# LeCAR-Lab/dial-mpc

Hardware: AMD Instinct MI355X
Metric: sample-rollouts/sec (N x H env.steps), Go2 N=2048 H=16 (higher is better)
Workload: dtype f32

## Files before the change

### dial_mpc_amd/_lib.py

```python
from __future__ import annotations

import ctypes
import glob
import os
import subprocess
from typing import Optional

import numpy as np

from dial_mpc_amd import _abi

_CSRC = os.path.join(os.path.dirname(os.path.abspath(__file__)), "csrc")
LIB_PATH = os.environ.get("DIAL_HIP_LIB", os.path.join(_CSRC, "libdialhip.so"))
_lib = None


class DialHipError(RuntimeError):
    pass


IEEE_LIB_PATH = os.path.join(_CSRC, "libdialhip_ieee.so")


N_FAMILIES = 8
_FAST = ["-DDIAL_FUSED_DPP", "-fno-hip-fp32-correctly-rounded-divide-sqrt", "-Xarch_device", "-freciprocal-math", "-Xarch_device", "-fapprox-func",
         "-Xarch_device", "-fno-honor-nans"]
_IEEE = ["-Xarch_device", "-ffp-contract=off", "-DDIAL_IEEE_BUILD"]
_COMMON = ["--offload-arch=gfx950", "-O3", "-std=c++17", "-fPIC", "-Xarch_device", "-fno-slp-vectorize"]
_FAMILY_FLAGS = {3: ["-mllvm", "-amdgpu-sched-strategy=max-ilp"], 4: ["-mllvm", "-simplifycfg-sink-common=false"]}


def build(force: bool = False, verbose: bool = False, ieee: bool = False) -> str:
    if not ieee:
        build_plant(force=force, verbose=verbose)
        build_plant_dist(force=force, verbose=verbose)
        build_plant_var(force=force, verbose=verbose)
        build_plan_var(force=force, verbose=verbose)
        build_plan_ens(force=force, verbose=verbose)
    return _build_lib(IEEE_LIB_PATH if ieee else LIB_PATH, [(os.path.join(_CSRC, "dial_hip.hip"), [], "dial_hip.o")] +
                      [(os.path.join(_CSRC, "kern_family.hip"), [f"-DDIAL_FAMILY={k}"] + _FAMILY_FLAGS.get(k, []), f"kern_family_{k}.o")
                       for k in range(N_FAMILIES)], force, verbose, ieee)


PLANT_LIB_PATH = os.path.join(_CSRC, "libdialplant.so")
N_PLANT_FAMILIES = 7


def build_plant(force: bool = False, verbose: bool = False) -> str:
    return _build_lib(PLANT_LIB_PATH, [(os.path.join(_CSRC, "plant_family.hip"), [f"-DDIAL_FAMILY={k}"] + _FAMILY_FLAGS.get(k, []),
                                        f"plant_family_{k}.o") for k in range(N_PLANT_FAMILIES)], force, verbose, False)


PLANT_DIST_LIB_PATH = os.path.join(_CSRC, "libdialplantdist.so")


def build_plant_dist(force: bool = False, verbose: bool = False) -> str:
    return _build_lib(PLANT_DIST_LIB_PATH, [(os.path.join(_CSRC, "plant_dist_family.hip"), [f"-DDIAL_FAMILY={k}"] + _FAMILY_FLAGS.get(k, []),
                                             f"plant_dist_family_{k}.o") for k in range(N_PLANT_FAMILIES)], force, verbose, False)


PLANT_VAR_LIB_PATH = os.path.join(_CSRC, "libdialplantvar.so")


def build_plant_var(force: bool = False, verbose: bool = False) -> str:
    return _build_lib(PLANT_VAR_LIB_PATH, [(os.path.join(_CSRC, "plant_var_family.hip"), [f"-DDIAL_FAMILY={k}"] + _FAMILY_FLAGS.get(k, []),
                                            f"plant_var_family_{k}.o") for k in range(N_PLANT_FAMILIES)], force, verbose, False)


PLAN_VAR_LIB_PATH = os.path.join(_CSRC, "libdialplanvar.so")


def build_plan_var(force: bool = False, verbose: bool = False) -> str:
    return _build_lib(PLAN_VAR_LIB_PATH, [(os.path.join(_CSRC, "plan_var_family.hip"), [f"-DDIAL_FAMILY={k}"] + _FAMILY_FLAGS.get(k, []),
                                           f"plan_var_family_{k}.o") for k in range(N_PLANT_FAMILIES)], force, verbose, False)


PLAN_ENS_LIB_PATH = os.path.join(_CSRC, "libdialplanens.so")


def build_plan_ens(force: bool = False, verbose: bool = False) -> str:
    return _build_lib(PLAN_ENS_LIB_PATH, [(os.path.join(_CSRC, "plan_ens_family.hip"), [f"-DDIAL_FAMILY={k}"] + _FAMILY_FLAGS.get(k, []),
                                           f"plan_ens_family_{k}.o") for k in range(N_PLANT_FAMILIES)] +
                      [(os.path.join(_CSRC, "plan_ens_aggregate.hip"), [], "plan_ens_aggregate.o")], force, verbose, False)


def _build_lib(out: str, units, force: bool, verbose: bool, ieee: bool) -> str:
    from concurrent.futures import ThreadPoolExecutor
    srcs = sorted(glob.glob(os.path.join(_CSRC, "*.h")) + glob.glob(os.path.join(_CSRC, "*.hip"))) + [_abi.HEADER, os.path.abspath(__file__)]
    if not force and os.path.exists(out) and all(os.path.getmtime(out) >= os.path.getmtime(s) for s in srcs):
        return out
    hipcc = os.environ.get("HIPCC", "/opt/rocm/bin/hipcc")
    flags = _COMMON + (_IEEE if ieee else _FAST) + ([] if ieee else os.environ.get("DIAL_HIPCC_EXTRA", "").split())
    import fcntl
    import hashlib
    import shutil
    build_root = os.path.join(os.path.dirname(os.path.dirname(_CSRC)), "build")
    os.makedirs(build_root, exist_ok=True)
    tag = hashlib.sha1(" ".join(flags).encode()).hexdigest()[:8]
    objdir = os.path.join(build_root, f"obj_{os.path.basename(out)}_{tag}_{os.getpid()}")
    tmp_out = f"{out}.{os.getpid()}.tmp"
    with open(os.path.join(build_root, os.path.basename(out) + ".lock"), "w") as lock:
        fcntl.flock(lock, fcntl.LOCK_EX)
        try:
            if not force and os.path.exists(out) and all(os.path.getmtime(out) >= os.path.getmtime(s) for s in srcs):
                return out
            os.makedirs(objdir, exist_ok=True)
            units = [(src, defs, os.path.join(objdir, obj)) for src, defs, obj in units]

            def compile_unit(u):
                src, defs, obj = u
                cmd = [hipcc] + flags + defs + ["-c", "-o", obj, src]
                if verbose:
                    print(" ".join(cmd))
                r = subprocess.run(cmd, stdout=subprocess.PIPE, stderr=subprocess.STDOUT, text=True)
                if r.returncode != 0:
                    raise DialHipError(f"hipcc failed ({r.returncode}) on {os.path.basename(src)} {' '.join(defs)}:\n{r.stdout[-4000:]}")
                return obj
            with ThreadPoolExecutor(max_workers=min(len(units), os.cpu_count() or 1, 16)) as pool:
                objs = list(pool.map(compile_unit, units))
            cmd = [hipcc, "--offload-arch=gfx950", "-shared", "-fPIC", "-o", tmp_out] + objs
            if verbose:
                print(" ".join(cmd))
            subprocess.check_call(cmd)
            os.replace(tmp_out, out)
            return out
        finally:
            shutil.rmtree(objdir, ignore_errors=True)
            if os.path.exists(tmp_out):
                os.remove(tmp_out)
            fcntl.flock(lock, fcntl.LOCK_UN)


def load(path: Optional[str] = None):
    global _lib
    if path is None and _lib is not None:
        return _lib
    lib_path = LIB_PATH if path is None else path
    if not os.path.exists(lib_path):
        raise DialHipError(f"{lib_path} is missing: run `python -c 'import __graft_entry__ as g; g.build()'` "
                           "(the HIP extension is the only compute path; there is no CPU fallback)")
    lib = ctypes.CDLL(lib_path)
    vp, ci, fp = ctypes.c_void_p, ctypes.c_int, ctypes.c_void_p
    lib.dial_create.argtypes = [ctypes.POINTER(vp), vp, vp, vp, ci]
    lib.dial_create_sharded.argtypes = [ctypes.POINTER(vp), vp, vp, vp, ci, ci]
    lib.dial_create_ex.argtypes = [ctypes.POINTER(vp), vp, vp, vp, ci, ci, vp]
    lib.dial_set_state_trace.argtypes = [vp, fp, ci]
    lib.dial_destroy.argtypes = [vp]
    lib.dial_destroy.restype = None
    lib.dial_last_error.argtypes = [vp]
    lib.dial_last_error.restype = ctypes.c_char_p
    lib.dial_rollout.argtypes = [vp, fp, fp, ci, fp, fp, fp, fp, vp]
    lib.dial_reverse_once.argtypes = [vp, fp, fp, fp, ci, fp, fp, fp, fp, fp, fp, vp]
    lib.dial_shard_rollout.argtypes = [vp, fp, fp, fp, ci, fp, ci, ci, fp, vp]
    lib.dial_shard_reduce.argtypes = [vp, fp, ci, ci, ci, ci, fp, vp]
    lib.dial_shard_ybar.argtypes = [vp, fp, ci, fp, fp, fp, ci, fp, vp]
    u64, u32 = ctypes.c_uint64, ctypes.c_uint32
    lib.dial_reverse_once_rng.argtypes = [vp, fp, fp, fp, ci, u64, u32, fp, fp, fp, fp, fp, vp]
# ... 570 lines not shown
        Y = Y.clone()
        self._check(self.lib.dial_shift_batch(self.h, _ptr(Y), int(Y.shape[0]), _stream()), "dial_shift_batch")
        return Y

    def rng_fill(self, seed: int, counter: int, n_begin: int, n_count: int):
        import torch
        eps = torch.empty((n_count, self.cfg.Hnode + 1, self.nu), dtype=torch.float32, device=self.torch_device)
        self._check(self.lib.dial_rng_fill(self.h, int(seed), int(counter), n_begin, n_count, _ptr(eps), _stream()),
                    "dial_rng_fill")
        return eps

    def shard_rollout_rng(self, state, Ybar, noise_scale, seed, counter, n_begin, n_local, with_mean, rews_local):
        self._check(self.lib.dial_shard_rollout_rng(self.h, _ptr(state), _ptr(Ybar), _ptr(noise_scale),
                                                    int(noise_scale.numel()), int(seed), int(counter), n_begin, n_local,
                                                    int(with_mean), _ptr(rews_local), _stream()), "dial_shard_rollout_rng")

    def shard_rollout(self, state, Ybar, noise_scale, eps_local, n_local: int, with_mean: bool, rews_local):
        ns = int(noise_scale.numel())
        self._check(self.lib.dial_shard_rollout(self.h, _ptr(state), _ptr(Ybar), _ptr(noise_scale), ns,
                                                _ptr(eps_local) if n_local > 0 else None, n_local, int(with_mean),
                                                _ptr(rews_local), _stream()), "dial_shard_rollout")

    def shard_reduce(self, rews_all, n_total: int, n_begin: int, n_local: int, include_mean: bool, packed_out):
        self._check(self.lib.dial_shard_reduce(self.h, _ptr(rews_all), n_total, n_begin, n_local, int(include_mean),
                                               _ptr(packed_out), _stream()), "dial_shard_reduce")

    def shard_ybar(self, rews_all, n_total: int, eps_all, Ybar, noise_scale, Ybar_out):
        ns = int(noise_scale.numel())
        self._check(self.lib.dial_shard_ybar(self.h, _ptr(rews_all), n_total, _ptr(eps_all), _ptr(Ybar), _ptr(noise_scale),
                                             ns, _ptr(Ybar_out), _stream()), "dial_shard_ybar")

    def shard_ybar_rng(self, rews_all, n_total: int, seed: int, counter: int, Ybar, noise_scale, Ybar_out):
        self._check(self.lib.dial_shard_ybar_rng(self.h, _ptr(rews_all), n_total, int(seed), int(counter), _ptr(Ybar),
                                                 _ptr(noise_scale), int(noise_scale.numel()), _ptr(Ybar_out), _stream()),
                    "dial_shard_ybar_rng")

    def shard_pack_rewards(self, gathered, world: int, per: int, n_total: int, rews_all):
        self._check(self.lib.dial_shard_pack_rewards(self.h, _ptr(gathered), world, per, n_total, _ptr(rews_all), _stream()),
                    "dial_shard_pack_rewards")

    def shard_ybar_gathered(self, gathered, world: int, per: int, n_total: int, eps_all, Ybar, noise_scale, rews_all, Ybar_out):
        self._check(self.lib.dial_shard_ybar_gathered(self.h, _ptr(gathered), world, per, n_total, _ptr(eps_all), _ptr(Ybar), _ptr(noise_scale),
                                                      int(noise_scale.numel()), _ptr(rews_all), _ptr(Ybar_out), _stream()), "dial_shard_ybar_gathered")

    def shard_ybar_gathered_rng(self, gathered, world: int, per: int, n_total: int, seed: int, counter: int, Ybar, noise_scale, rews_all, Ybar_out):
        self._check(self.lib.dial_shard_ybar_gathered_rng(self.h, _ptr(gathered), world, per, n_total, int(seed), int(counter), _ptr(Ybar),
                                                          _ptr(noise_scale), int(noise_scale.numel()), _ptr(rews_all), _ptr(Ybar_out), _stream()),
                    "dial_shard_ybar_gathered_rng")

    def shard_reduce_gathered(self, gathered, world: int, per: int, n_total: int, n_begin: int, n_local: int, include_mean: bool, rews_all, packed_out):
        self._check(self.lib.dial_shard_reduce_gathered(self.h, _ptr(gathered), world, per, n_total, n_begin, n_local, int(include_mean),
                                                        _ptr(rews_all), _ptr(packed_out), _stream()), "dial_shard_reduce_gathered")

    def packed_size(self) -> int:
        T, Hn1 = self.cfg.Hsample + 1, self.cfg.Hnode + 1
        return Hn1 * self.nu + T * (self.nq + self.nv + self.nx)

    def shift(self, Y):
        Y = Y.clone()
        self._check(self.lib.dial_shift(self.h, _ptr(Y), _stream()), "dial_shift")
        return Y

    def status(self):
        self._check(self.lib.dial_status(self.h), "dial_status")

    def set_timing(self, enable: bool):
        self._check(self.lib.dial_set_timing(self.h, int(enable)), "dial_set_timing")

    def rollout_ms(self):
        tot, n = ctypes.c_double(0), ctypes.c_int(0)
        self._check(self.lib.dial_get_rollout_ms(self.h, ctypes.byref(tot), ctypes.byref(n)), "dial_get_rollout_ms")
        return tot.value, n.value

    def set_state_trace(self, rows: Optional[int]):
        import torch
        if rows is None:
            self._check(self.lib.dial_set_state_trace(self.h, None, 0), "dial_set_state_trace")
            self._trace = None
            return None
        self._trace = torch.zeros((int(rows), self.cfg.Hsample + 1, self.state_size), dtype=torch.float32, device=self.torch_device)
        self._check(self.lib.dial_set_state_trace(self.h, _ptr(self._trace), int(rows)), "dial_set_state_trace")
        return self._trace

    LAUNCH_FIELDS = ("inst", "wpb", "blocks", "queue", "relay", "mean_inline", "slice_pieces", "split", "pair", "trace", "con_cap", "rollouts")

    def debug_last_launch(self) -> dict:
        buf = (ctypes.c_int * len(self.LAUNCH_FIELDS))()
        n = self.lib.dial_debug_last_launch(self.h, buf, len(buf))
        if n != len(self.LAUNCH_FIELDS):
            raise DialHipError(f"dial_debug_last_launch: {n} fields, this wrapper knows {len(self.LAUNCH_FIELDS)}")
        return dict(zip(self.LAUNCH_FIELDS, buf))

    def debug_scratch(self):
        import numpy as np
        import torch
        ptrs = [ctypes.c_void_p() for _ in range(6)]
        self._check(self.lib.dial_debug_scratch(self.h, *[ctypes.byref(p) for p in ptrs]), "dial_debug_scratch")
        cfg = self.cfg
        B, T, Hn1 = cfg.Nsample + 1, cfg.Hsample + 1, cfg.Hnode + 1
        shapes = [(B, Hn1, self.nu), (B, T), (B, T, self.nq), (B, T, self.nv), (B, T, self.nx), (B,)]
        names = ["Y0s", "rewss", "qss", "qdss", "xss", "weights"]
        torch.cuda.synchronize()
        hip = ctypes.CDLL("libamdhip64.so")
        out = {}
        for name, p, shp in zip(names, ptrs, shapes):
            host = np.empty(shp, np.float32)
            rc = hip.hipMemcpy(host.ctypes.data_as(ctypes.c_void_p), p, ctypes.c_size_t(host.nbytes), ctypes.c_int(2))
            if rc != 0:
                raise DialHipError(f"hipMemcpy of scratch {name} failed ({rc})")
            out[name] = host
        return out
```

### dial_mpc_amd/csrc/dial_hip.hip

```cpp
#include <dlfcn.h>
#include <hip/hip_runtime.h>

#include <cstdio>
#include <cstdlib>
#include <cstring>
#include <string>
#include <vector>

#include "kernel_list.h"
#include "plant_kernel.h"
#include "plant_plugin.h"
#include "plant_dist_kernel.h"
#include "plant_var_kernel.h"
#include "plan_var_kernel.h"
#include "plan_ens_kernel.h"
#include "plugin_ops.h"

#define DIAL_X(D, WPB, OCC, Q, TR) \
  extern template __global__ void rollout_kernel<D, WPB, OCC, Q, TR>(const CModel<D>*, const dial_task*, const dial_cfg*, dial::RolloutIO, int, int, int*);
#define DIAL_XE(D)                                                                                                                                    \
  extern template __global__ void env_step_kernel<D>(const CModel<D>*, const dial_task*, float*, const float*, float*, float*, float*, const float*); \
  extern template __global__ void env_reset_kernel<D>(const CModel<D>*, const float*, const float*, float*, float*, float*);
DIAL_KERNELS_ALL(DIAL_X, DIAL_XE)
#define DIAL_X2(D, WPB, OCC, Q, MI) \
  extern template __global__ void rollout_kernel2<D, WPB, OCC, Q, MI>(const CModel<D>*, const dial_task*, const dial_cfg*, dial::RolloutIO, int, int, int*);
DIAL_KERNELS2_GO2(DIAL_X2)
#undef DIAL_X2
#undef DIAL_X
#undef DIAL_XE

#define WSUM_CHUNKS 64
#define YB_CHUNKS_HOST 128

#ifndef DIAL_GO2_LARGE_B
#define DIAL_GO2_LARGE_B 2304
#endif
#ifndef DIAL_GO2_PAIR_MIN_B
#define DIAL_GO2_PAIR_MIN_B 2304
#endif

#define WK_THREADS 1024
#ifndef DIAL_K4_FP64
#define DIAL_K4_FP64 0
#endif
__device__ __forceinline__ float block_sum(float v, float* red) {
  const int tid = threadIdx.x;
  float ws = dialwave::wave_sum_dpp(v);
  if ((tid & 63) == 0) red[tid >> 6] = ws;
  __syncthreads();
  float r = 0.f;
#pragma unroll
  for (int k = 0; k < WK_THREADS / 64; k++) r += red[k];
  __syncthreads();
  return r;
}
__device__ __forceinline__ double block_sum_d(double v, double* red) {
  const int tid = threadIdx.x;
  for (int o = 32; o > 0; o >>= 1) v += __shfl_xor(v, o, 64);
  if ((tid & 63) == 0) red[tid >> 6] = v;
  __syncthreads();
  double r = 0.0;
#pragma unroll
  for (int k = 0; k < WK_THREADS / 64; k++) r += red[k];
  __syncthreads();
  return r;
}
__device__ __forceinline__ float block_max(float v, float* red) {
  const int tid = threadIdx.x;
  float wm = dialwave::wave_max_shfl(v);
  if ((tid & 63) == 0) red[tid >> 6] = wm;
  __syncthreads();
  float r = -INFINITY;
#pragma unroll
  for (int k = 0; k < WK_THREADS / 64; k++) r = red[k] > r ? red[k] : r;
  __syncthreads();
  return r;
}

extern "C" __global__ void __launch_bounds__(WK_THREADS)
weights_kernel(const float* __restrict__ rews_in, int B, float temp, float* __restrict__ weights, const float* __restrict__ gathered,
               int per, float* __restrict__ rews_out) {
  __shared__ float red[WK_THREADS / 64];
  const int tid = threadIdx.x;
  const float* rews = rews_in + (size_t)blockIdx.x * B;
  weights += (size_t)blockIdx.x * B;
  if (gathered) {
    const int n_total = B - 1;
    for (int n = tid; n < B; n += WK_THREADS)
      rews_out[n] = n < n_total ? gathered[(size_t)(n / per) * (per + 1) + (n % per)] : gathered[per];
    __threadfence_block();
    __syncthreads();
    rews = rews_out;
  }
#if DIAL_K4_FP64
  __shared__ double redd[WK_THREADS / 64];
  double accd = 0.0;
  float mxr = -INFINITY;
  for (int n = tid; n < B; n += WK_THREADS) { float r = rews[n]; accd += (double)r; mxr = r > mxr ? r : mxr; }
  const double mean = block_sum_d(accd, redd) / (double)B;
// ... 103 lines not shown
        if (eps) {
#pragma unroll
          for (int e = 0; e < 4; e++) z[e] = c0 + e < C ? eps[(size_t)n * C + c0 + e] : 0.f;
        } else {
          dial::normal_quad((uint32_t)n, (uint32_t)q, iter, seed_lo, seed_hi, z);
        }
      }
      const float wn = weights[n];
#pragma unroll
      for (int e = 0; e < 4; e++) {
        float v = n < n_total ? (kk[e] == 0 ? y0[e] : z[e] * sc[e] + yb[e]) : yb[e];
        v = v < -1.f ? -1.f : (v > 1.f ? 1.f : v);
        acc[e] += wn * v;
      }
    }
  }
#pragma unroll
  for (int e = 0; e < 4; e++) red[rl][4 * ql + e] = acc[e];
  __syncthreads();
  const int cl = threadIdx.x, c = blockIdx.x * 64 + cl;
  if (cl < 64 && c < C) {
    float t = 0.f;
    for (int r = 0; r < 16; r++) t += red[r][cl];
    partial[(size_t)chunk * C + c] = t;
  }
}
extern "C" __global__ void __launch_bounds__(64)
ybar_final_kernel(const float* __restrict__ partial, int C, float* __restrict__ out) {
  const int c = blockIdx.x * 64 + threadIdx.x;
  if (c >= C) return;
  float acc = 0.f;
#pragma unroll 16
  for (int ch = 0; ch < YB_CHUNKS; ch++) acc += partial[(size_t)ch * C + c];
  out[c] = acc;
}

extern "C" __global__ void __launch_bounds__(256)
rng_fill_kernel(uint32_t seed_lo, uint32_t seed_hi, uint32_t iter, int n_begin, int n_count, int C, float* eps_out) {
  const int nq = (C + 3) / 4;
  const long long t = (long long)blockIdx.x * 256 + threadIdx.x;
  if (t >= (long long)n_count * nq) return;
  const int n = (int)(t / nq), q = (int)(t - (long long)n * nq);
  float z[4];
  dial::normal_quad((uint32_t)(n_begin + n), (uint32_t)q, iter, seed_lo, seed_hi, z);
  for (int e = 0; e < 4; e++)
    if (4 * q + e < C) eps_out[(size_t)n * C + 4 * q + e] = z[e];
}

extern "C" __global__ void __launch_bounds__(256)
pack_rewards_kernel(const float* __restrict__ gathered, int per, int n_total, float* __restrict__ rews_all) {
  const int n = blockIdx.x * 256 + threadIdx.x;
  if (n < n_total) rews_all[n] = gathered[(size_t)(n / per) * (per + 1) + (n % per)];
  else if (n == n_total) rews_all[n] = gathered[per];
}

extern "C" __global__ void __launch_bounds__(64)
shift_kernel(const dial_cfg* __restrict__ cfg, int nu, float* Y) {
  __shared__ float u[DIAL_MAX_T * DIAL_MAX_U];
  const int T = cfg->Hsample + 1, Hn1 = cfg->Hnode + 1;
  Y += (size_t)blockIdx.x * Hn1 * nu;
  for (int it = threadIdx.x; it < T * nu; it += 64) {
    const int st = it / nu, a = it - st * nu;
    float acc = 0.f;
    if (st + 1 < T)
      for (int k = 0; k < Hn1; k++) acc += cfg->W[st + 1][k] * Y[k * nu + a];
    u[it] = acc;
  }
  __syncthreads();
  for (int it = threadIdx.x; it < Hn1 * nu; it += 64) {
    const int k = it / nu, a = it - k * nu;
    float acc = 0.f;
    for (int st = 0; st < T; st++) acc += cfg->V[k][st] * u[st * nu + a];
    Y[it] = acc;
  }
}

extern "C" __global__ void __launch_bounds__(64) selftest_kernel(float* out) {
  float v = (float)threadIdx.x + 0.5f;
  float a = dialwave::wave_sum_dpp(v), b = dialwave::wave_sum_shfl(v), c = dialwave::wave_max_shfl(v);
  if (threadIdx.x == 0) { out[0] = a; out[1] = b; out[2] = c; }
}

enum LaunchField { LF_INST, LF_WPB, LF_BLOCKS, LF_QUEUE, LF_RELAY, LF_MEAN_INLINE, LF_SLICE_PIECES, LF_SPLIT, LF_PAIR, LF_TRACE, LF_CON_CAP,
                   LF_ROLLOUTS, DIAL_LAUNCH_FIELDS };

struct dial_ctx {
  int device = 0;
  dial_model hm;
  dial_task ht;
  dial_cfg hc;
  dial_derived hd;
  bool has_cfg = false;
  int inst = 0;
  const dial_plugin_ops* plug = nullptr;
  const dial_plugin_ctrl* plug_ctrl = nullptr;
  const dial_plugin_table* plug_table = nullptr;
  const dial_plugin_plant* plug_plant = nullptr;
  const dial_plugin_plant_dist* plug_plant_dist = nullptr;
  const float* plant_dist = nullptr;
  int plant_dist_M = 0, plant_dist_E = 0;
  const dial_plugin_plant_var* plug_plant_var = nullptr;
  void* plant_models = nullptr;
  int32_t* plant_model_of = nullptr;
  int plant_models_V = 0, plant_models_M = 0;
  const dial_plugin_plan_var* plug_plan_var = nullptr;
  void* plan_models = nullptr;
  int32_t* plan_model_of = nullptr;
  int plan_models_V = 0, plan_models_rows = 0, plan_models_mode = 0;
  dial_plan_var_launch_fn plan_launch = nullptr;
  const dial_plugin_plan_ens* plug_plan_ens = nullptr;
  void* ens_models = nullptr;
  int32_t* ens_hyp = nullptr;
  float* ens_raw = nullptr;
  int ens_V = 0, ens_rows = 0, ens_R = 0, ens_mode = 0, ens_k = 0;
  int ens_last_M = 0;
  dial_plan_ens_launch_fn ens_launch = nullptr;
  dial_plan_ens_aggregate_fn ens_aggregate = nullptr;
  std::vector<float> user_params;
  const float* user_table = nullptr;
  int user_table_rows = 0, user_table_cols = 0, user_table_row0 = 0, user_table_mode = 0;
  std::vector<char> plug_cm;
  const float* plan_params = nullptr;
  int plan_rows = 0;
  void* dcm = nullptr;
  size_t dcm_bytes = 0;
  dial_task* dtask = nullptr;
  dial_cfg* dcfg = nullptr;
  int con_cap = 0, ovf_words = 0;
  float* ovf = nullptr;
  int B_cap = 0, W_cap = 0, T = 0, Hn1 = 0, nx = 0;
  int plan_cap = 1;
  float *Y0s = nullptr, *rewss = nullptr, *rews = nullptr, *qss = nullptr, *qdss = nullptr, *xss = nullptr;
  float *weights = nullptr, *partial = nullptr;
  const char* rows_stale = nullptr;
  unsigned long long* prof = nullptr;
  size_t lds_bytes = 0;
  size_t lds_rollout = 0;
  size_t lds_large = 0;
  int ws_words = 0, cm_bytes = 0, wpb = 1;
  int* next = nullptr;
  float* relay_buf = nullptr;
  float* slice_buf = nullptr;
  int* slice_flag = nullptr;
  int slice_cap = 0, slice_stride = 0, slice_steps = 3;
  int* work_stat = nullptr;
  int* relay_flag = nullptr;
  int* err_host = nullptr;
  int* err_dev = nullptr;
  bool relay_ok = false, relay_always = false;
  bool no_spread = false;
  bool no_mean_inline = false;
  hipStream_t side = nullptr;
  hipEvent_t ev_fork = nullptr, ev_join = nullptr;
  size_t lds_even = 0, lds_one = 0;
  bool split_ok = false;
  int wpb_even = 0;
  int n_simd = 0;
  int debug_stall_piece1 = 0;
  int relay_steps = 3;
  int resident_blocks = 0, resident_blocks_large = 0;
  bool pair_ok = false;
  size_t lds_pair = 0, lds_pair_large = 0;
  int resident_pair = 0, resident_pair_large = 0;
  bool timing = false;
  dial_options opt{};
  float* trace = nullptr;
  int trace_rows = 0;
  int ovf_slots = 0;
  int last_launch[DIAL_LAUNCH_FIELDS] = {};
  std::vector<std::pair<hipEvent_t, hipEvent_t>> events;
  size_t events_used = 0;
  std::string err;
};

static thread_local std::string g_err;

static int fail(dial_ctx* ctx, int code, const std::string& msg) {
  if (ctx) ctx->err = msg;
  g_err = msg;
  return code;
}
#define HIP_TRY(ctx, expr)                                                                     \
  do {                                                                                         \
    hipError_t e_ = (expr);                                                                    \
    if (e_ != hipSuccess)                                                                      \
      return fail(ctx, DIAL_ERR_HIP, std::string(#expr) + ": " + hipGetErrorString(e_));       \
  } while (0)

template <class Tab>
static int plugin_table(void* h, const char* plugin_path, const char* symbol, const char* what, int version, const Tab** tab) {
  typedef const Tab* (*entry_fn)(void);
  *tab = nullptr;
  entry_fn entry = (entry_fn)dlsym(h, symbol);
  if (!entry) return DIAL_OK;
  *tab = entry();
  if (!*tab) return fail(nullptr, DIAL_ERR_ARG, std::string("dial_create_plugin: ") + plugin_path + ": " + symbol + " returned no table");
  if ((*tab)->version != version)
    return fail(nullptr, DIAL_ERR_ARG, std::string("dial_create_plugin: stale plugin: its ") + what + " reports version " + std::to_string((*tab)->version) +
                                       ", the library needs version " + std::to_string(version) + " (rebuild it from the current sources)");
  return DIAL_OK;
}

template <class D>
static void plant_model_block(void* dst, const dial_model* model, const dial_task* task, const dial_derived* dv) {
  CModel<D>* h = new CModel<D>();
  fill_cmodel(h, model, task, dv);
  memcpy(dst, h, sizeof(CModel<D>));
  delete h;
}

extern "C" {

const char* dial_last_error(const dial_ctx* ctx) { return ctx ? ctx->err.c_str() : g_err.c_str(); }

int dial_abi_sizes(int* a, int* b, int* c) {
  if (a) *a = (int)sizeof(dial_model);
  if (b) *b = (int)sizeof(dial_task);
  if (c) *c = (int)sizeof(dial_cfg);
  return DIAL_OK;
}

void dial_destroy(dial_ctx* ctx) {
  if (!ctx) return;
  (void)hipSetDevice(ctx->device);
  void* ptrs[] = {ctx->dcm, ctx->dtask, ctx->dcfg, ctx->prof, ctx->next, ctx->relay_buf, ctx->relay_flag, ctx->Y0s, ctx->rewss, ctx->rews, ctx->qss,
                  ctx->qdss,   ctx->xss,   ctx->weights, ctx->partial, ctx->ovf, ctx->slice_buf, ctx->slice_flag, ctx->work_stat,
                  ctx->plant_models, ctx->plant_model_of, ctx->plan_models, ctx->plan_model_of, ctx->ens_models, ctx->ens_hyp, ctx->ens_raw};
  for (void* p : ptrs)
    if (p) (void)hipFree(p);
  for (auto& ev : ctx->events) { (void)hipEventDestroy(ev.first); (void)hipEventDestroy(ev.second); }
  if (ctx->ev_fork) (void)hipEventDestroy(ctx->ev_fork);
  if (ctx->ev_join) (void)hipEventDestroy(ctx->ev_join);
  if (ctx->side) (void)hipStreamDestroy(ctx->side);
  if (ctx->err_host) (void)hipHostFree(ctx->err_host);
  delete ctx;
}

int dial_create(dial_ctx** out, const dial_model* model, const dial_task* task, const dial_cfg* cfg, int device) {
  return dial_create_ex(out, model, task, cfg, device, -1, nullptr);
}

int dial_create_sharded(dial_ctx** out, const dial_model* model, const dial_task* task, const dial_cfg* cfg, int device,
                        int n_local_cap) {
  if (cfg && (n_local_cap < 0 || n_local_cap > cfg->Nsample)) return fail(nullptr, DIAL_ERR_ARG, "dial_create_sharded: n_local_cap must be in [0, Nsample]");
  return dial_create_ex(out, model, task, cfg, device, n_local_cap, nullptr);
}

static int create_impl(dial_ctx** out, const dial_model* model, const dial_task* task, const dial_cfg* cfg, int device,
                       int n_local_cap, const dial_options* opts, const dial_plugin_ops* plug, const float* params, int n_params);

int dial_create_ex(dial_ctx** out, const dial_model* model, const dial_task* task, const dial_cfg* cfg, int device,
                   int n_local_cap, const dial_options* opts) {
  return create_impl(out, model, task, cfg, device, n_local_cap, opts, nullptr, nullptr, 0);
}

int dial_create_plugin(dial_ctx** out, const dial_model* model, const dial_task* task, const dial_cfg* cfg, int device,
                       const dial_options* opts, const char* plugin_path, const float* params, int n_params) {
  if (!out || !model || !task || !plugin_path) return fail(nullptr, DIAL_ERR_ARG, "dial_create_plugin: null argument");
// ... 310 lines not shown
      case 3: ctx->inst = 3; ctx->wpb = 2; urc = upload(DimsH1Loco{}); break;
      case 4: ctx->inst = 4; ctx->wpb = DIAL_ALLEGRO_WPB; urc = upload(DimsAllegro{}); break;
      case 5: ctx->inst = 5; ctx->wpb = DIAL_CRATE_WPB; urc = upload(DimsGo2Crate{}); break;
      case 6: ctx->inst = 6; ctx->wpb = DIAL_CRATE_WPB; urc = upload(DimsH1PushCrate{}); break;
      case 0: ctx->inst = 0; ctx->wpb = 1; urc = upload(DimsMax{}); break;
      default:
        dial_destroy(ctx);
        return fail(nullptr, DIAL_ERR_UNSUPPORTED, std::string("dial_create: elliptic-cone models need a dimension-specialised instantiation (built: Allegro hand)") +
                                                   (opt.force_generic ? "; options.force_generic does not apply to them" : ""));
    }
    if (urc != DIAL_OK) { dial_destroy(ctx); return fail(nullptr, urc, "dial_create: uploading the model constants failed"); }
    ctx->last_launch[LF_INST] = ctx->inst;
  }
  if (!cfg) ctx->lds_rollout = ctx->lds_bytes;
  if (ctx->lds_rollout > 160 * 1024 || ctx->lds_bytes > 64 * 1024) {
    dial_destroy(ctx);
    return fail(nullptr, DIAL_ERR_ARG, "dial_create: LDS workspace exceeds the 160 KiB of a CU");
  }
  if (ctx->inst == 1) ctx->lds_large = ctx->cm_bytes + (size_t)DIAL_GO2_WPB_LARGE * ctx->ws_words * sizeof(float);
  {
    hipError_t e = hipSuccess;
    if (ctx->inst == 4 && ctx->lds_rollout > 64 * 1024)
      e = hipFuncSetAttribute((const void*)rollout_kernel<DimsAllegro, DIAL_ALLEGRO_WPB>, hipFuncAttributeMaxDynamicSharedMemorySize, (int)ctx->lds_rollout);
    if (e == hipSuccess && ctx->inst == 4 && ctx->lds_rollout > 64 * 1024)
      e = hipFuncSetAttribute((const void*)rollout_kernel<DimsAllegro, DIAL_ALLEGRO_WPB, 3, true>, hipFuncAttributeMaxDynamicSharedMemorySize, (int)ctx->lds_rollout);
    if (e == hipSuccess && ctx->inst == 4 && ctx->lds_rollout > 64 * 1024)
      e = hipFuncSetAttribute((const void*)rollout_kernel<DimsAllegro, DIAL_ALLEGRO_WPB, 3, false, true>, hipFuncAttributeMaxDynamicSharedMemorySize, (int)ctx->lds_rollout);
#define DIAL_BIG_LDS(D)                                                                                                                         \
    if (e == hipSuccess && ctx->lds_rollout > 64 * 1024) {                                                                                     \
      e = hipFuncSetAttribute((const void*)rollout_kernel<D, DIAL_CRATE_WPB>, hipFuncAttributeMaxDynamicSharedMemorySize, (int)ctx->lds_rollout); \
      if (e == hipSuccess) e = hipFuncSetAttribute((const void*)rollout_kernel<D, DIAL_CRATE_WPB, 3, true>, hipFuncAttributeMaxDynamicSharedMemorySize, (int)ctx->lds_rollout); \
      if (e == hipSuccess) e = hipFuncSetAttribute((const void*)rollout_kernel<D, DIAL_CRATE_WPB, 3, false, true>, hipFuncAttributeMaxDynamicSharedMemorySize, (int)ctx->lds_rollout); \
    }
    if (ctx->inst == 7) e = ctx->plug->set_lds(ctx->lds_rollout);
    if (ctx->inst == 5) { DIAL_BIG_LDS(DimsGo2Crate) }
    if (ctx->inst == 6) { DIAL_BIG_LDS(DimsH1PushCrate) }
#undef DIAL_BIG_LDS
    if (e == hipSuccess && ctx->inst == 1 && ctx->lds_large > 64 * 1024)
      e = hipFuncSetAttribute((const void*)rollout_kernel<DimsGo2, DIAL_GO2_WPB_LARGE, DIAL_GO2_OCC_LARGE, true>, hipFuncAttributeMaxDynamicSharedMemorySize, (int)ctx->lds_large);
    if (ctx->inst == 1 && cfg) {
      ctx->pair_ok = opt.pair_mode != 1;
      ctx->lds_pair = ctx->cm_bytes + (size_t)2 * ctx->ws_words * sizeof(float);
      ctx->lds_pair_large = ctx->cm_bytes + (size_t)2 * DIAL_GO2_PAIR_WPB * ctx->ws_words * sizeof(float);
#ifdef DIAL_PROFILE
      ctx->lds_pair += 16 + 32 * sizeof(unsigned long long);
      ctx->lds_pair_large += 16 + (size_t)DIAL_GO2_PAIR_WPB * 32 * sizeof(unsigned long long);
#endif
      if (ctx->lds_pair_large > 160 * 1024) ctx->pair_ok = false;
      if (e == hipSuccess && ctx->pair_ok && ctx->lds_pair_large > 64 * 1024)
        e = hipFuncSetAttribute((const void*)rollout_kernel2<DimsGo2, DIAL_GO2_PAIR_WPB, DIAL_GO2_PAIR_OCC, true, true>, hipFuncAttributeMaxDynamicSharedMemorySize, (int)ctx->lds_pair_large);
    }
    if (e != hipSuccess) { dial_destroy(ctx); return fail(nullptr, DIAL_ERR_HIP, std::string("dial_create: hipFuncSetAttribute: ") + hipGetErrorString(e)); }
  }
  {
    hipDeviceProp_t prop;
    HIP_TRY_CREATE(hipGetDeviceProperties(&prop, device));
    int nb = 0;
    hipError_t e = hipSuccess;
#define DIAL_RESIDENT(D, WPB) e = hipOccupancyMaxActiveBlocksPerMultiprocessor(&nb, rollout_kernel<D, WPB>, 64 * WPB, ctx->lds_rollout)
    if (ctx->inst == 1) DIAL_RESIDENT(DimsGo2, 1);
    else if (ctx->inst == 2) DIAL_RESIDENT(DimsH1, 3);
    else if (ctx->inst == 3) DIAL_RESIDENT(DimsH1Loco, 2);
    else if (ctx->inst == 4) DIAL_RESIDENT(DimsAllegro, DIAL_ALLEGRO_WPB);
    else if (ctx->inst == 5) DIAL_RESIDENT(DimsGo2Crate, DIAL_CRATE_WPB);
    else if (ctx->inst == 6) DIAL_RESIDENT(DimsH1PushCrate, DIAL_CRATE_WPB);
    else if (ctx->inst == 7) e = ctx->plug->occupancy(&nb, ctx->lds_rollout);
    else DIAL_RESIDENT(DimsMax, 1);
#undef DIAL_RESIDENT
    ctx->n_simd = 4 * prop.multiProcessorCount;
    if (e == hipSuccess) ctx->resident_blocks = nb * prop.multiProcessorCount;
    if (e == hipSuccess && ctx->inst == 1) {
      e = hipOccupancyMaxActiveBlocksPerMultiprocessor(&nb, rollout_kernel<DimsGo2, DIAL_GO2_WPB_LARGE, DIAL_GO2_OCC_LARGE, true>,
                                                       64 * DIAL_GO2_WPB_LARGE, ctx->lds_large);
      if (e == hipSuccess) ctx->resident_blocks_large = nb * prop.multiProcessorCount;
    }
    if (e == hipSuccess && ctx->pair_ok) {
      e = hipOccupancyMaxActiveBlocksPerMultiprocessor(&nb, rollout_kernel2<DimsGo2, 1, DIAL_GO2_PAIR_OCC, false, false>, 64, ctx->lds_pair);
      if (e == hipSuccess) ctx->resident_pair = nb * prop.multiProcessorCount;
      if (e == hipSuccess) e = hipOccupancyMaxActiveBlocksPerMultiprocessor(&nb, rollout_kernel2<DimsGo2, DIAL_GO2_PAIR_WPB, DIAL_GO2_PAIR_OCC, true, true>,
                                                                            64 * DIAL_GO2_PAIR_WPB, ctx->lds_pair_large);
      if (e == hipSuccess) ctx->resident_pair_large = nb * prop.multiProcessorCount;
      if (e == hipSuccess && (ctx->resident_pair <= 0 || ctx->resident_pair_large <= 0)) ctx->pair_ok = false;
    }
    if (e != hipSuccess) { dial_destroy(ctx); return fail(nullptr, DIAL_ERR_HIP, std::string("dial_create: occupancy query: ") + hipGetErrorString(e)); }
    if (opt.no_queue) ctx->resident_blocks = ctx->resident_blocks_large = 0;
    HIP_TRY_CREATE(hipMalloc(&ctx->next, sizeof(int)));
    HIP_TRY_CREATE(hipMalloc(&ctx->relay_buf, sizeof(float) * (DIAL_MAX_Q + 2 * DIAL_MAX_V + DIAL_INFO_N + 4)));
    HIP_TRY_CREATE(hipMalloc(&ctx->relay_flag, sizeof(int)));
    HIP_TRY_CREATE(hipMemset(ctx->relay_flag, 0, sizeof(int)));
    HIP_TRY_CREATE(hipHostMalloc((void**)&ctx->err_host, sizeof(int), hipHostMallocMapped));
    *ctx->err_host = 0;
    HIP_TRY_CREATE(hipHostGetDevicePointer((void**)&ctx->err_dev, ctx->err_host, 0));
    ctx->relay_ok = ctx->wpb == 1 && !opt.no_relay;
    ctx->relay_always = opt.relay_always != 0;
    ctx->no_mean_inline = opt.no_mean_inline != 0;
    ctx->no_spread = opt.no_spread != 0;
    ctx->wpb_even = ctx->inst == 4 ? DIAL_ALLEGRO_WPB_EVEN : ctx->inst == 2 ? DIAL_H1_WPB_EVEN : 0;
    if ((opt.no_split_mask >> ctx->inst) & 1) ctx->wpb_even = 0;
    if (ctx->wpb_even > 0) {
      ctx->lds_even = ctx->cm_bytes + (size_t)ctx->wpb_even * ctx->ws_words * sizeof(float);
      ctx->lds_one = ctx->cm_bytes + (size_t)ctx->ws_words * sizeof(float);
#ifdef DIAL_PROFILE
      ctx->lds_even += 16 + (size_t)ctx->wpb_even * 32 * sizeof(unsigned long long);
      ctx->lds_one += 16 + 32 * sizeof(unsigned long long);
#endif
      if ((8 / ctx->wpb_even) * ctx->lds_even + ctx->lds_one <= 160 * 1024) {
        hipError_t e2 = hipSuccess;
        if (ctx->lds_even > 64 * 1024) {
          if (ctx->inst == 4) e2 = hipFuncSetAttribute((const void*)rollout_kernel<DimsAllegro, DIAL_ALLEGRO_WPB_EVEN, DIAL_EVEN_OCC_ALLEGRO>, hipFuncAttributeMaxDynamicSharedMemorySize, (int)ctx->lds_even);
          else e2 = hipFuncSetAttribute((const void*)rollout_kernel<DimsH1, DIAL_H1_WPB_EVEN, DIAL_EVEN_OCC_H1>, hipFuncAttributeMaxDynamicSharedMemorySize, (int)ctx->lds_even);
        }
        if (e2 == hipSuccess) e2 = hipStreamCreateWithFlags(&ctx->side, hipStreamNonBlocking);
        if (e2 == hipSuccess) e2 = hipEventCreateWithFlags(&ctx->ev_fork, hipEventDisableTiming);
        if (e2 == hipSuccess) e2 = hipEventCreateWithFlags(&ctx->ev_join, hipEventDisableTiming);
        if (e2 != hipSuccess) { dial_destroy(ctx); return fail(nullptr, DIAL_ERR_HIP, std::string("dial_create: split-launch set-up: ") + hipGetErrorString(e2)); }
        ctx->split_ok = true;
      }
    }
    if (opt.relay_steps >= 1) ctx->relay_steps = opt.relay_steps;
    ctx->debug_stall_piece1 = opt.debug_relay_stall;
  }
  HIP_TRY_CREATE(hipMalloc(&ctx->dtask, sizeof(dial_task)));
  HIP_TRY_CREATE(hipMemcpy(ctx->dtask, task, sizeof(dial_task), hipMemcpyHostToDevice));
  if (cfg) {
    if (cfg->Hsample + 1 > DIAL_MAX_T || cfg->Hnode + 1 > DIAL_MAX_NODE || cfg->Hnode < 2 || cfg->Nsample < 1) {
      dial_destroy(ctx);
      return fail(nullptr, DIAL_ERR_ARG, "dial_create: Hsample/Hnode/Nsample out of range");
    }
    ctx->hc = *cfg;
    ctx->has_cfg = true;
    ctx->B_cap = n_local_cap + 1;
    ctx->W_cap = cfg->Nsample + 1;
    ctx->ovf_slots = ctx->plan_cap * ctx->B_cap + (cfg->Hsample + 1 > 16 ? cfg->Hsample + 1 : 16);
    if (ctx->con_cap > 0) HIP_TRY_CREATE(hipMalloc(&ctx->ovf, (size_t)ctx->ovf_slots * ctx->ovf_words * sizeof(float)));
    ctx->T = cfg->Hsample + 1;
    ctx->Hn1 = cfg->Hnode + 1;
    if (ctx->inst == 4 && !opt.no_lag_priority) HIP_TRY_CREATE(hipMalloc(&ctx->work_stat, 2 * sizeof(int)));
    const int B_all = ctx->plan_cap * ctx->B_cap;
    if (ctx->inst == 4 && !opt.no_slice && ctx->resident_blocks > 0 && B_all > ctx->resident_blocks * ctx->wpb) {
      ctx->slice_stride = model->nq + 2 * model->nv + DIAL_INFO_N + 4;
      ctx->slice_cap = B_all;
      if (opt.slice_steps >= 1) ctx->slice_steps = opt.slice_steps;
      HIP_TRY_CREATE(hipMalloc(&ctx->slice_buf, sizeof(float) * (size_t)ctx->slice_stride * B_all));
      HIP_TRY_CREATE(hipMalloc(&ctx->slice_flag, sizeof(int) * (size_t)B_all));
      HIP_TRY_CREATE(hipMemset(ctx->slice_flag, 0, sizeof(int) * (size_t)B_all));
    }
    const size_t B = B_all, T = ctx->T;
    HIP_TRY_CREATE(hipMalloc(&ctx->dcfg, sizeof(dial_cfg)));
    HIP_TRY_CREATE(hipMemcpy(ctx->dcfg, cfg, sizeof(dial_cfg), hipMemcpyHostToDevice));
    HIP_TRY_CREATE(hipMalloc(&ctx->Y0s, sizeof(float) * B * ctx->Hn1 * model->nu));
    HIP_TRY_CREATE(hipMalloc(&ctx->rewss, sizeof(float) * B * T));
    HIP_TRY_CREATE(hipMalloc(&ctx->rews, sizeof(float) * ctx->W_cap));
    HIP_TRY_CREATE(hipMalloc(&ctx->qss, sizeof(float) * B * T * model->nq));
    HIP_TRY_CREATE(hipMalloc(&ctx->qdss, sizeof(float) * B * T * model->nv));
    HIP_TRY_CREATE(hipMalloc(&ctx->xss, sizeof(float) * B * T * ctx->nx));
    HIP_TRY_CREATE(hipMalloc(&ctx->weights, sizeof(float) * ctx->W_cap * ctx->plan_cap));
    const size_t Ctot = (size_t)ctx->Hn1 * model->nu + T * (model->nq + model->nv + ctx->nx);
    const size_t part_w = ((Ctot + 63) / 64) * (size_t)WSUM_CHUNKS * 64, part_y = (((size_t)ctx->Hn1 * model->nu + 63) / 64) * (size_t)YB_CHUNKS_HOST * 64;
    HIP_TRY_CREATE(hipMalloc(&ctx->partial, sizeof(float) * (part_w * ctx->plan_cap > part_y ? part_w * ctx->plan_cap : part_y)));
    HIP_TRY_CREATE(hipMalloc(&ctx->prof, sizeof(unsigned long long) * (32 + 6 * B)));
    HIP_TRY_CREATE(hipMemset(ctx->prof, 0, sizeof(unsigned long long) * (32 + 6 * B)));
  }
#undef HIP_TRY_CREATE
  *out = ctx;
  return DIAL_OK;
}
// ... 132 lines not shown
    if ((B + 1) / 2 <= ctx->resident_pair || opt_no_queue(ctx)) {
      const int pairs = (B + 1) / 2;
      ll[LF_PAIR] = 1; ll[LF_WPB] = 1; ll[LF_BLOCKS] = pairs;
      hipLaunchKernelGGL((rollout_kernel2<DimsGo2, 1, DIAL_GO2_PAIR_OCC, false, false>), dim3(pairs), dim3(64), ctx->lds_pair, st,
                         (const CModel<DimsGo2>*)ctx->dcm, (const dial_task*)ctx->dtask, (const dial_cfg*)ctx->dcfg, io, B, ctx->ws_words, (int*)nullptr);
    } else {
      const int blocks = ctx->resident_pair_large;
      if (mean_last && ctx->T <= blocks * DIAL_GO2_PAIR_WPB) {
        io.mean_inline = 1;
        io.relay_buf = ctx->relay_buf;
        io.relay_flag = ctx->relay_flag;
        io.err_word = ctx->err_dev;
      }
      HIP_TRY(ctx, hipMemsetD32Async((hipDeviceptr_t)ctx->next, blocks * DIAL_GO2_PAIR_WPB, 1, st));
      ll[LF_PAIR] = 1; ll[LF_WPB] = DIAL_GO2_PAIR_WPB; ll[LF_BLOCKS] = blocks; ll[LF_QUEUE] = 1; ll[LF_MEAN_INLINE] = io.mean_inline;
      hipLaunchKernelGGL((rollout_kernel2<DimsGo2, DIAL_GO2_PAIR_WPB, DIAL_GO2_PAIR_OCC, true, true>), dim3(blocks), dim3(64 * DIAL_GO2_PAIR_WPB),
                         ctx->lds_pair_large, st, (const CModel<DimsGo2>*)ctx->dcm, (const dial_task*)ctx->dtask, (const dial_cfg*)ctx->dcfg, io, B,
                         ctx->ws_words, ctx->next);
    }
    HIP_TRY(ctx, hipGetLastError());
    if (ctx->timing) HIP_TRY(ctx, hipEventRecord(e1, st));
    return DIAL_OK;
  }
  const bool large = ctx->inst == 1 && B > DIAL_GO2_LARGE_B && !tracing;
  const int wpb = large ? DIAL_GO2_WPB_LARGE : ctx->wpb;
  const int resident = large ? ctx->resident_blocks_large : ctx->resident_blocks;
  dial::RolloutIO io = io_in;
  io.plan_params = ctx->plan_params;
  io.con_cap = ctx->ovf ? ctx->con_cap : 0;
  io.ovf = ctx->ovf;
  io.ovf_words = ctx->ovf_words;
  bool relay = false;
  if (ctx->relay_ok && !large && !io.us && !io.plan_rollouts && io.n_noise == B - 1 && B > 1 && ctx->T >= 4 && ctx->n_simd > 0 &&
      ((B - 1) % ctx->n_simd == 0 || ctx->relay_always)) {
    const int pieces = (ctx->T + ctx->relay_steps - 1) / ctx->relay_steps;
    if ((B - 1) + pieces <= ctx->resident_blocks) {
      io.relay_buf = ctx->relay_buf;
      io.relay_flag = ctx->relay_flag;
      io.relay_steps = ctx->relay_steps;
      io.relay_base = B - 1;
      io.err_word = ctx->err_dev;
      io.debug_stall_piece1 = ctx->debug_stall_piece1;
      relay = true;
    }
  }
  int blocks = io.relay_flag ? io.relay_base + (ctx->T + io.relay_steps - 1) / io.relay_steps : (B + wpb - 1) / wpb;
  if (large && !io.relay_flag && resident > 0 && blocks < resident && !ctx->no_spread) {
    blocks = resident;
    io.spread = 1;
  }
  int* next = nullptr;
  const bool has_queue_variant = large || ctx->inst != 1;
  if (has_queue_variant && resident > 0 && blocks > resident && ctx->next && !tracing) {
    blocks = resident;
    next = ctx->next;
    HIP_TRY(ctx, hipMemsetD32Async((hipDeviceptr_t)next, blocks * wpb, 1, st));
    if (large && !ctx->no_mean_inline && !io.us && !io.plan_rollouts && io.n_noise == B - 1 && ctx->T <= blocks * wpb && io.relay_stride == 0) {
      io.mean_inline = 1;
      io.relay_buf = ctx->relay_buf;
      io.relay_flag = ctx->relay_flag;
      io.err_word = ctx->err_dev;
    }
    if (!io.mean_inline && ctx->slice_buf && B <= ctx->slice_cap && ctx->T > ctx->slice_steps) {
      io.relay_buf = ctx->slice_buf;
      io.relay_flag = ctx->slice_flag;
      io.relay_stride = ctx->slice_stride;
      io.relay_steps = ctx->slice_steps;
      io.slice_pieces = (ctx->T + ctx->slice_steps - 1) / ctx->slice_steps;
      io.err_word = ctx->err_dev;
    }
  }
  if (ctx->work_stat && !io.slice_pieces && !tracing) {
    HIP_TRY(ctx, hipMemsetAsync(ctx->work_stat, 0, 2 * sizeof(int), st));
    io.work_stat = ctx->work_stat;
  }
  if (io.ovf && blocks * wpb > ctx->ovf_slots)
    return fail(ctx, DIAL_ERR_ARG, "rollout launch: more wavefronts than overflow areas (batch larger than the context's Nsample + 1)");
  if (ctx->trace) {
    if (B > ctx->trace_rows) return fail(ctx, DIAL_ERR_ARG, "rollout launch: more rollouts than rows of the state trace (dial_set_state_trace)");
    io.trace = ctx->trace;
  }
  ll[LF_WPB] = wpb; ll[LF_BLOCKS] = blocks; ll[LF_QUEUE] = next != nullptr; ll[LF_RELAY] = relay; ll[LF_MEAN_INLINE] = io.mean_inline;
  ll[LF_SLICE_PIECES] = io.slice_pieces; ll[LF_TRACE] = tracing; ll[LF_CON_CAP] = io.con_cap;
  if (ctx->split_ok && !tracing && !next && !io.us && !io.plan_rollouts && io.n_noise == B - 1 && (B - 1) == 8 * (ctx->n_simd / 4)) {
    HIP_TRY(ctx, hipEventRecord(ctx->ev_fork, st));
    HIP_TRY(ctx, hipStreamWaitEvent(ctx->side, ctx->ev_fork, 0));
    dial::RolloutIO io1 = io;
    io1.n_first = B - 1;
    ll[LF_SPLIT] = 1; ll[LF_WPB] = ctx->wpb_even; ll[LF_BLOCKS] = (B - 1) / ctx->wpb_even;
#define DIAL_SPLIT_LAUNCH(D, WPBE, OCCE)                                                                                       \
    hipLaunchKernelGGL((rollout_kernel<D, 1>), dim3(1), dim3(64), ctx->lds_one, ctx->side, (const CModel<D>*)ctx->dcm,     \
                       (const dial_task*)ctx->dtask, (const dial_cfg*)ctx->dcfg, io1, B, ctx->ws_words, (int*)nullptr);    \
    HIP_TRY(ctx, hipGetLastError());                                                                                       \
    HIP_TRY(ctx, hipEventRecord(ctx->ev_join, ctx->side));                                                                 \
    hipLaunchKernelGGL((rollout_kernel<D, WPBE, OCCE>), dim3((B - 1) / WPBE), dim3(64 * WPBE), ctx->lds_even, st,                \
                       (const CModel<D>*)ctx->dcm, (const dial_task*)ctx->dtask, (const dial_cfg*)ctx->dcfg, io, B - 1,    \
                       ctx->ws_words, (int*)nullptr)
    if (ctx->inst == 4) { DIAL_SPLIT_LAUNCH(DimsAllegro, DIAL_ALLEGRO_WPB_EVEN, DIAL_EVEN_OCC_ALLEGRO); }
    else { DIAL_SPLIT_LAUNCH(DimsH1, DIAL_H1_WPB_EVEN, DIAL_EVEN_OCC_H1); }
#undef DIAL_SPLIT_LAUNCH
    HIP_TRY(ctx, hipGetLastError());
    HIP_TRY(ctx, hipStreamWaitEvent(st, ctx->ev_join, 0));
    if (ctx->timing) HIP_TRY(ctx, hipEventRecord(e1, st));
    return DIAL_OK;
  }
#define DIAL_LAUNCH_ROLLOUT_Q(D, WPB, Q)                                                                    \
  hipLaunchKernelGGL((rollout_kernel<D, WPB, 3, Q>), dim3(blocks), dim3(64 * WPB), ctx->lds_rollout,        \
                     st, (const CModel<D>*)ctx->dcm, (const dial_task*)ctx->dtask,                          \
                     (const dial_cfg*)ctx->dcfg, io, B, ctx->ws_words, next)
#define DIAL_LAUNCH_ROLLOUT(D, WPB)                                        \
  do {                                                                     \
    if (next) DIAL_LAUNCH_ROLLOUT_Q(D, WPB, true);                         \
    else DIAL_LAUNCH_ROLLOUT_Q(D, WPB, false);                             \
  } while (0)
#define DIAL_LAUNCH_TRACE(D, WPB)                                                                           \
  hipLaunchKernelGGL((rollout_kernel<D, WPB, 3, false, true>), dim3(blocks), dim3(64 * WPB), ctx->lds_rollout, \
                     st, (const CModel<D>*)ctx->dcm, (const dial_task*)ctx->dtask,                          \
                     (const dial_cfg*)ctx->dcfg, io, B, ctx->ws_words, (int*)nullptr)
  if (tracing) {
    if (ctx->inst == 1) DIAL_LAUNCH_TRACE(DimsGo2, 1);
    else if (ctx->inst == 2) DIAL_LAUNCH_TRACE(DimsH1, 3);
    else if (ctx->inst == 3) DIAL_LAUNCH_TRACE(DimsH1Loco, 2);
    else if (ctx->inst == 4) DIAL_LAUNCH_TRACE(DimsAllegro, DIAL_ALLEGRO_WPB);
    else if (ctx->inst == 5) DIAL_LAUNCH_TRACE(DimsGo2Crate, DIAL_CRATE_WPB);
    else if (ctx->inst == 6) DIAL_LAUNCH_TRACE(DimsH1PushCrate, DIAL_CRATE_WPB);
    else if (ctx->inst == 7) HIP_TRY(ctx, ctx->plug->rollout(2, blocks, ctx->lds_rollout, st, ctx->dcm, ctx->dtask, ctx->dcfg, &io, B, ctx->ws_words, nullptr));
    else DIAL_LAUNCH_TRACE(DimsMax, 1);
  } else
  if (large)
    hipLaunchKernelGGL((rollout_kernel<DimsGo2, DIAL_GO2_WPB_LARGE, DIAL_GO2_OCC_LARGE, true>), dim3(blocks),
                       dim3(64 * DIAL_GO2_WPB_LARGE), ctx->lds_large, st, (const CModel<DimsGo2>*)ctx->dcm, (const dial_task*)ctx->dtask,
                       (const dial_cfg*)ctx->dcfg, io, B, ctx->ws_words, next);
  else if (ctx->inst == 1) DIAL_LAUNCH_ROLLOUT_Q(DimsGo2, 1, false);
  else if (ctx->inst == 2) DIAL_LAUNCH_ROLLOUT(DimsH1, 3);
  else if (ctx->inst == 3) DIAL_LAUNCH_ROLLOUT(DimsH1Loco, 2);
  else if (ctx->inst == 4) DIAL_LAUNCH_ROLLOUT(DimsAllegro, DIAL_ALLEGRO_WPB);
  else if (ctx->inst == 5) DIAL_LAUNCH_ROLLOUT(DimsGo2Crate, DIAL_CRATE_WPB);
  else if (ctx->inst == 6) DIAL_LAUNCH_ROLLOUT(DimsH1PushCrate, DIAL_CRATE_WPB);
  else if (ctx->inst == 7) HIP_TRY(ctx, ctx->plug->rollout(next ? 1 : 0, blocks, ctx->lds_rollout, st, ctx->dcm, ctx->dtask, ctx->dcfg, &io, B, ctx->ws_words, next));
  else DIAL_LAUNCH_ROLLOUT(DimsMax, 1);
#undef DIAL_LAUNCH_ROLLOUT
#undef DIAL_LAUNCH_ROLLOUT_Q
#undef DIAL_LAUNCH_TRACE
  HIP_TRY(ctx, hipGetLastError());
  if (ctx->timing) HIP_TRY(ctx, hipEventRecord(e1, st));
  return DIAL_OK;
}

int dial_rollout(dial_ctx* ctx, const float* state, const float* us, int B, float* rewss, float* qss, float* qdss,
                 float* xposs, void* stream) {
  if (!ctx || !state || !us || !rewss || B < 1) return fail(ctx, DIAL_ERR_ARG, "dial_rollout: bad argument");
  if (!ctx->has_cfg) return fail(ctx, DIAL_ERR_ARG, "dial_rollout: context was created without a dial_cfg");
  HIP_TRY(ctx, hipSetDevice(ctx->device));
  dial::RolloutIO io{state, us, nullptr, nullptr, nullptr, 0, 0, ctx->T, ctx->Hn1, nullptr, rewss, nullptr, qss, qdss, xposs, nullptr, 0, 0u, 0u, 0u, 0};
  return launch_rollout(ctx, io, B, (hipStream_t)stream);
}

static int shard_rollout_impl(dial_ctx* ctx, const float* state, const float* Ybar_in, const float* noise_scale,
                              int ns, const float* eps, int use_rng, uint64_t seed, uint32_t counter, int n_begin,
                              int n_local, int with_mean, float* rews_local, void* stream, const char* who,
                              bool store_states = true) {
  if (!ctx || !state || !Ybar_in || !noise_scale || (!eps && !use_rng && n_local > 0) || !rews_local)
    return fail(ctx, DIAL_ERR_ARG, std::string(who) + ": null argument");
  if (!ctx->has_cfg) return fail(ctx, DIAL_ERR_ARG, std::string(who) + ": context was created without a dial_cfg");
  if (ns != 1 && ns != ctx->Hn1) return fail(ctx, DIAL_ERR_ARG, std::string(who) + ": noise_scale must have 1 or Hnode+1 entries");
  if (with_mean & ~3) return fail(ctx, DIAL_ERR_ARG, std::string(who) + ": with_mean = " + std::to_string(with_mean) + " is outside 0 .. 3");
  if (with_mean & 2) store_states = false;
  const bool lean = (with_mean & 2) != 0;
  with_mean &= 1;
  const int B = n_local + (with_mean ? 1 : 0);
  if (n_local < 0 || B < 1 || B > ctx->B_cap || n_begin < 0) return fail(ctx, DIAL_ERR_ARG, std::string(who) + ": shard larger than Nsample+1");
  HIP_TRY(ctx, hipSetDevice(ctx->device));
  dial::RolloutIO io{state, nullptr, eps, Ybar_in, noise_scale, ns, n_local, ctx->T, ctx->Hn1,
                     lean ? nullptr : ctx->Y0s, ctx->rewss, rews_local, store_states ? ctx->qss : nullptr, store_states ? ctx->qdss : nullptr,
                     store_states ? ctx->xss : nullptr, ctx->prof,
                     use_rng, (uint32_t)(seed & 0xffffffffu), (uint32_t)(seed >> 32), counter, n_begin};
  if (lean) ctx->rows_stale = "the last rollout launch was lean (DIAL_SHARD_LEAN): it wrote neither the candidate nodes nor the per-step states";
  else if (!store_states) ctx->rows_stale = "the last rollout launch formed the mean action only (reverse_once without bars): it wrote no per-step states";
  const int rc = launch_rollout(ctx, io, B, (hipStream_t)stream);
  if (rc == DIAL_OK && store_states) ctx->rows_stale = nullptr;
  return rc;
}

int dial_shard_rollout(dial_ctx* ctx, const float* state, const float* Ybar_in, const float* noise_scale, int ns,
                       const float* eps, int n_local, int with_mean, float* rews_local, void* stream) {
  if (ctx && ctx->plug) return fail(ctx, DIAL_ERR_ARG, "dial_shard_rollout: sharded use of a task-plugin context is not supported");
  return shard_rollout_impl(ctx, state, Ybar_in, noise_scale, ns, eps, 0, 0, 0, 0, n_local, with_mean, rews_local,
                            stream, "dial_shard_rollout");
}

int dial_shard_rollout_rng(dial_ctx* ctx, const float* state, const float* Ybar_in, const float* noise_scale, int ns,
                           uint64_t seed, uint32_t counter, int n_begin, int n_local, int with_mean,
                           float* rews_local, void* stream) {
  if (ctx && ctx->plug) return fail(ctx, DIAL_ERR_ARG, "dial_shard_rollout_rng: sharded use of a task-plugin context is not supported");
  return shard_rollout_impl(ctx, state, Ybar_in, noise_scale, ns, nullptr, 1, seed, counter, n_begin, n_local,
                            with_mean, rews_local, stream, "dial_shard_rollout_rng");
}

int dial_rng_fill(dial_ctx* ctx, uint64_t seed, uint32_t counter, int n_begin, int n_count, float* eps_out,
                  void* stream) {
  if (!ctx || !eps_out || n_count < 0 || n_begin < 0) return fail(ctx, DIAL_ERR_ARG, "dial_rng_fill: bad argument");
  if (!ctx->has_cfg) return fail(ctx, DIAL_ERR_ARG, "dial_rng_fill: context was created without a dial_cfg");
  if (n_count == 0) return DIAL_OK;
  HIP_TRY(ctx, hipSetDevice(ctx->device));
  const int C = ctx->Hn1 * ctx->hm.nu, nq = (C + 3) / 4;
  const long long total = (long long)n_count * nq;
  hipLaunchKernelGGL(rng_fill_kernel, dim3((unsigned)((total + 255) / 256)), dim3(256), 0, (hipStream_t)stream,
                     (uint32_t)(seed & 0xffffffffu), (uint32_t)(seed >> 32), counter, n_begin, n_count, C, eps_out);
  HIP_TRY(ctx, hipGetLastError());
  return DIAL_OK;
}

static int launch_wsum(dial_ctx* ctx, const float* weights, int n_rows, int w_begin, int mean_row, int mean_widx,
                       float* Yo, float* qo, float* qdo, float* xo, hipStream_t st, bool nodes_only = false, int plans = 1) {
  const dial_model& m = ctx->hm;
// ... 999 lines not shown
```

### dial_mpc_amd/csrc/rollout_body.h

```cpp
#pragma once
#include "derived.h"
#include "dmath.h"

#define MJ_MINVAL 1e-15f
#define MJ_MINIMP 0.0001f
#define MJ_MAXIMP 0.9999f
#define DIAL_PI 3.14159265358979323846f

namespace dial {

template <class D>
inline constexpr bool kNeedL = D::gen;

struct RowRef { int is_lim, dof, c, tan; float f; };
template <class M>
DIAL_DEV int con_of(const M*, const Ws& s, int c) {
  if constexpr (!M::D::gen) return c;
  else return (int)s.clist[c];
}
template <class M>
DIAL_DEV RowRef row_ref(const M* m, const Ws& s, int r) {
  RowRef rr;
  const int nl = dim_nl(m), nlf = nl + dim_nf(m);
  rr.is_lim = r < nlf;
// ... 1496 lines not shown
      constexpr int NV = M::D::NV, S = M::D::S;
      w.items(NV * S / 4, [&](int e) {
        const int i = (4 * e) / S, j0 = 4 * e - i * S;
        float a = s.M[4 * e], b = s.M[4 * e + 1], c2 = s.M[4 * e + 2], d2 = s.M[4 * e + 3];
        const float add = dt * m->dof_damping[i];
        const int dj = i - j0;
        a += dj == 0 ? add : 0.f; b += dj == 1 ? add : 0.f; c2 += dj == 2 ? add : 0.f; d2 += dj == 3 ? add : 0.f;
        store4(s.H + 4 * e, a, b, c2, d2);
      });
      const vfloat rhs = w.per_lane([&](int l) { return l < NV ? s.qfs[l] + s.qfc[l] : 0.f; });
      const vfloat x = reg_chol<typename M::D>(w, m, s.H, rhs, s.H);
      w.items(NV, [&](int i) { s.qvel[i] += lane_val(x, i) * dt; });
    } else {
      w.items(dim_nv(m), [&](int i) { s.qvel[i] += s.qacc[i] * dt; });
    }
  } else if constexpr (M::D::pre_ctrl) {
    float* qdrow = nullptr;
    if (w.out_io && w.out_io->qdss) qdrow = w.out_io->qdss + (size_t)w.out_row * dim_nv(m);
    w.items(dim_nv(m), [&](int i) {
      const float v = s.qvel[i] + s.qacc[i] * dt;
      s.qvel[i] = v;
      if (qdrow) qdrow[i] = v;
    });
  } else
  w.items(dim_nv(m), [&](int i) { s.qvel[i] += s.qacc[i] * dt; });
  w.items(dim_nj(m), [&](int ji) {
    const int qa = m->jnt_qposadr[ji], da = m->jnt_dofadr[ji];
    if (m->jnt_type[ji] == DIAL_JNT_FREE) {
      for (int k = 0; k < 3; k++) s.qpos[qa + k] += dt * s.qvel[da + k];
      float v[3] = {s.qvel[da + 3], s.qvel[da + 4], s.qvel[da + 5]};
      const float w2 = dm::dot3(v, v);
      float nrm = w2 >= DM_FLT_MIN ? DM_SQRT(w2) : 0.f, axis[3] = {1.f, 0.f, 0.f}, qr[4], qn[4];
      if (nrm > 0.f) { axis[0] = v[0] / nrm; axis[1] = v[1] / nrm; axis[2] = v[2] / nrm; }
      dm::axis_angle_to_quat(qr, axis, dt * nrm);
      float q0[4] = {s.qpos[qa + 3], s.qpos[qa + 4], s.qpos[qa + 5], s.qpos[qa + 6]};
      dm::quat_mul(qn, q0, qr);
      dm::normalize4(qn);
      for (int k = 0; k < 4; k++) s.qpos[qa + 3 + k] = qn[k];
    } else {
      s.qpos[qa] += dt * s.qvel[da];
    }
  });
}

DIAL_DEV float foot_step_height(float tt, float footphase, float duty) {
  const float two_pi = 2.f * DIAL_PI;
  float x = tt + DIAL_PI - footphase;
  float angle = x - two_pi * DM_FLOOR(x / two_pi) - DIAL_PI;
  if (duty < 1.f) angle = angle * 0.5f / (1.f - duty);
  float clipped = dm::clip(angle, -DIAL_PI / 2.f, DIAL_PI / 2.f);
  float value = duty < 1.f ? DM_COS(clipped) : 0.f;
  return dm::absf(value) >= 1e-6f ? dm::absf(value) : 0.f;
}
DIAL_DEV float quat_yaw(const float* q) {
  return DM_ATAN2(-2.f * q[1] * q[2] + 2.f * q[0] * q[3], q[1] * q[1] + q[0] * q[0] - q[3] * q[3] - q[2] * q[2]);
}

template <class M>
DIAL_DEV float act2joint(const M* m, float act, int a) {
  float an = (act * m->action_scale + 1.0f) / 2.0f;
  float jt = (m->joint_range[a][0] + m->joint_offset[a]) + an * (m->joint_range[a][1] - m->joint_range[a][0]);
  return dm::clip(jt, m->phys_range[a][0], m->phys_range[a][1]);
}
DIAL_DEV int table_row_index(int step, int row0, int rows, int mode) {
  const int r = step + row0;
  if (mode == DIAL_TABLE_WRAP) { const int q = r % rows; return q < 0 ? q + rows : q; }
  return r < 0 ? 0 : (r > rows - 1 ? rows - 1 : r);
}
DIAL_DEV int table_next_index(int idx, int r_next, int rows, int mode) {
  if (mode == DIAL_TABLE_WRAP) return idx + 1 == rows ? 0 : idx + 1;
  return r_next < 0 ? 0 : (r_next > rows - 1 ? rows - 1 : r_next);
}
template <class M>
DIAL_DEV DialControlIn control_in(const M* m, float step, const float* qpos, const float* qvel, const float* act, const float* trow,
                                  int tindex) {
  return DialControlIn{dim_nq(m), dim_nv(m), dim_nu(m), step, m->dt, qpos, qvel, act, m->act_qposadr, m->act_dofadr, m->action_scale,
                       m->kp, m->kd, &m->joint_range[0][0], &m->phys_range[0][0], &m->tau_range[0][0], m->joint_offset,
                       trow, tindex, m->table, m->table_rows, m->table_cols};
}
template <class M>
DIAL_DEV float gait_ztar(const M* m, int f, float step) {
  return m->gait_amp * foot_step_height(step * m->dt * 2.f * DIAL_PI * m->gait_cadence + DIAL_PI, 2.f * DIAL_PI * m->gait_phase[f], m->gait_duty);
}
template <bool FULL_INFO, bool PRE = false, class W, class M>
DIAL_DEV float env_step(W& w, const M* m, const dial_task* tg, const Ws& s, int st = 0) {
  const int nu = dim_nu(m);
  const bool walk = m->kind == DIAL_TASK_GO2_WALK || m->kind == DIAL_TASK_H1_WALK || m->kind == DIAL_TASK_H1_LOCO ||
                    m->kind == DIAL_TASK_H1_PUSH_CRATE;
  static_assert(!PRE || M::D::pre_ctrl, "control tables: carved for the Dims::pre_ctrl instantiations only");
  if constexpr (PRE) {
    w.jrow = s.jtab + st * nu;
  } else if constexpr (M::D::user_ctrl) {
    w.items(nu, [&](int a) {
      const bool tab = m->table_rows > 0;
      const DialControlIn in = control_in(m, s.info[DIAL_INFO_STEP], s.qpos, s.qvel, s.act, tab ? m->table_ring[m->table_half] : nullptr,
                                          tab ? m->table_cur : 0);
      const float c = dial_user_control(in, a, m->user_params, s.info + DIAL_INFO_USER);
      s.ctrl[a] = c;
      s.info[DIAL_INFO_LAST_CTRL + a] = c;
    });
  } else
  w.items(nu + DIAL_MAX_FEET, [&](int it) {
    if (it < nu) {
      const int a = it;
      const float jt = act2joint(m, s.act[a], a);
      float c;
      if (m->position_control) c = jt;
      else {
        float q_err = jt - s.qpos[7 + a];
        c = dm::clip(m->kp[a] * q_err - m->kd[a] * s.qvel[6 + a], m->tau_range[a][0], m->tau_range[a][1]);
      }
      s.ctrl[a] = c;
    } else {
      const int f = it - nu;
      if (walk && f < m->nfeet) s.ztar[f] = gait_ztar(m, f, s.info[DIAL_INFO_STEP]);
    }
  });
  DIAL_MARK(w, 25);
  const int n_frames = PRE ? 1 : m->n_frames;
  for (int f = 0; f < n_frames; f++) {
#ifndef DIAL_EMU
    if (w.launder) { asm volatile("" : "+v"(w.lane)); w.lane_r = w.lane; }
#endif
    forward(w, m, s);
    euler(w, m, s);
    DIAL_MARK(w, 9);
  }
  if constexpr (M::D::user) {
    w.items(1, [&](int) {
      float* info = s.info;
      const float step = info[DIAL_INFO_STEP];
      const bool tab = m->table_rows > 0;
      const DialRewardIn in{dim_nq(m), dim_nv(m), nu, dim_nb(m), dim_ns(m), dim_nc(m), step, m->dt,
                            s.qpos, s.qvel, s.xpos, s.xquat, s.spos, s.cdist, s.cpos, s.ctrl, s.act,
                            tab ? m->table_ring[m->table_half] : nullptr, tab ? m->table_cur : 0, m->table, m->table_rows, m->table_cols};
      const float reward = dial_user_reward(in, m->user_params, info + DIAL_INFO_USER);
      if (FULL_INFO) info[DIAL_INFO_DONE] = 0.f;
      info[DIAL_INFO_STEP] = step + 1.f;
      info[DIAL_INFO_REWARD] = reward;
    });
    DIAL_MARK(w, 10);
    return s.info[DIAL_INFO_REWARD];
  }
  if (m->kind == DIAL_TASK_ALLEGRO) {
    w.items(3, [&](int it) {
      const int ob = m->torso_x + 1;
      float acc = 0.f;
      if (it == 0) {
        for (int k = 0; k < 3; k++) { const float e = s.cvel[6 * ob + k] * DIAL_PI / 180.0f - s.info[DIAL_INFO_ANG_VEL_TAR + k]; acc += e * e; }
      } else if (it == 1) {
        for (int k = 0; k < 3; k++) { const float e = s.xpos[3 * ob + k] - s.info[DIAL_INFO_POS_TAR + k]; acc += e * e; }
      } else {
        for (int a = 0; a < nu; a++) { const float e = s.qpos[7 + a] - m->joint_offset[a]; acc += e * e; }
      }
      s.rpart[it] = acc;
    });
    w.items(1, [&](int) {
      const float step = s.info[DIAL_INFO_STEP];
      const float reward = -s.rpart[0] * 1.0f + -s.rpart[1] * 5.0f + -s.rpart[2] * 0.1f;
      if (FULL_INFO) s.info[DIAL_INFO_DONE] = step >= 100.f ? 1.f : 0.f;
      s.info[DIAL_INFO_STEP] = step + 1.f;
      s.info[DIAL_INFO_REWARD] = reward;
    });
    DIAL_MARK(w, 10);
    return s.info[DIAL_INFO_REWARD];
  }
  if constexpr (M::D::gen && ((task_kind_mask<typename M::D>() >> DIAL_TASK_GO2_CRATE) & 1u)) {
    if (m->kind == DIAL_TASK_GO2_CRATE) {
      w.items(1, [&](int) {
        float* info = s.info;
        const int tb = m->torso_x + 1, ub = m->upright_x + 1;
        const float step = info[DIAL_INFO_STEP], dt = m->dt;
        const float tq[4] = {s.xquat[4 * tb], s.xquat[4 * tb + 1], s.xquat[4 * tb + 2], s.xquat[4 * tb + 3]};
        const float uq[4] = {s.xquat[4 * ub], s.xquat[4 * ub + 1], s.xquat[4 * ub + 2], s.xquat[4 * ub + 3]};
        const float hv[3] = {m->head_vec[0], m->head_vec[1], m->head_vec[2]};
        float mat[9], head[3];
        dm::quat_to_mat(mat, tq);
        float reward_pos = 0.f;
        for (int k = 0; k < 3; k++) {
          head[k] = s.xpos[3 * tb + k] + (mat[3 * k] * hv[0] + mat[3 * k + 1] * hv[1] + mat[3 * k + 2] * hv[2]);
          const float e = head[k] - (info[DIAL_INFO_POS_TAR + k] + info[DIAL_INFO_VEL_TAR + k] * dt * step);
          reward_pos += e * e;
        }
        const float up[3] = {0.f, 0.f, 1.f};
        float vec[3];
        dm::rotate(vec, up, uq);
        const float reward_upright = -((vec[0] - 0.f) * (vec[0] - 0.f) + (vec[1] - 0.f) * (vec[1] - 0.f) + (vec[2] - 1.f) * (vec[2] - 1.f));
        const float ey = quat_yaw(tq) - info[DIAL_INFO_YAW_TAR];
        float reward_contact = 0.f;
        for (int i = 0; i < 4; i++) {
          const float* cp = s.cpos + 3 * m->crate_contact[i];
          const bool cond = cp[0] > m->crate_region[0] && cp[0] < m->crate_region[1] && cp[1] > m->crate_region[2] &&
                            cp[1] < m->crate_region[3] && cp[2] > m->crate_region[4] && cp[2] < m->crate_region[5];
          reward_contact += cond ? 1.f : 0.f;
        }
        const float reward = -reward_pos * 1.0f + reward_upright * 0.01f + -(ey * ey) * 0.3f + reward_contact * 0.02f;
        if (FULL_INFO) info[DIAL_INFO_DONE] = 0.f;
        info[DIAL_INFO_STEP] = step + 1.f;
        info[DIAL_INFO_REWARD] = reward;
      });
      DIAL_MARK(w, 10);
      return s.info[DIAL_INFO_REWARD];
    }
  }
  auto reward_phase = [&](auto KIND) {
    constexpr int kind = decltype(KIND)::value;
    constexpr bool walk = kind == DIAL_TASK_GO2_WALK || kind == DIAL_TASK_H1_WALK || kind == DIAL_TASK_H1_LOCO ||
                          kind == DIAL_TASK_H1_PUSH_CRATE;
    constexpr int NF = (kind == DIAL_TASK_GO2_WALK || kind == DIAL_TASK_GO2_SEQ_JUMP) ? 4 : 2;
    auto term = [&](auto IT, const float* cmd) -> float {
      constexpr int it = decltype(IT)::value;
      const float dt = m->dt;
      const int tb = m->torso_x + 1, ub = m->upright_x + 1;
      float* info = s.info;
      const float step = info[DIAL_INFO_STEP];
      const float tq[4] = {s.xquat[4 * tb], s.xquat[4 * tb + 1], s.xquat[4 * tb + 2], s.xquat[4 * tb + 3]};
      const float uq[4] = {s.xquat[4 * ub], s.xquat[4 * ub + 1], s.xquat[4 * ub + 2], s.xquat[4 * ub + 3]};
      const float tp[3] = {s.xpos[3 * tb], s.xpos[3 * tb + 1], s.xpos[3 * tb + 2]};
      const float* cmr = s.com + 3 * m->body_rootid[tb];
      const float tcom[3] = {cmr[0], cmr[1], cmr[2]};
      const float tv[6] = {s.cvel[6 * tb], s.cvel[6 * tb + 1], s.cvel[6 * tb + 2], s.cvel[6 * tb + 3], s.cvel[6 * tb + 4], s.cvel[6 * tb + 5]};
      const float yaw_tar0 = info[DIAL_INFO_YAW_TAR], pos_tar_z = info[DIAL_INFO_POS_TAR + 2];
      float out = 0.f;
      if (it == 0) {
        if (walk) {
          float reward_gaits = 0.f;
  #pragma unroll
          for (int f = 0; f < NF; f++) {
            const float z_tar = PRE ? s.ztab[st * DIAL_ZTAB_W + f] : s.ztar[f], zs = s.spos[3 * m->feet_site[f] + 2];
            float fz;
            if (kind == DIAL_TASK_GO2_WALK) {
              float e = (z_tar - zs) / 0.05f;
              reward_gaits += e * e;
              fz = zs - m->foot_radius;
            } else if constexpr (kind == DIAL_TASK_H1_PUSH_CRATE) {
              float zf = dm::fminf_(s.cdist[pc_foot_contact(m, f, 0)], s.cdist[pc_foot_contact(m, f, 1)]);
              reward_gaits += (z_tar - zf) * (z_tar - zf);
              fz = zs;
            } else if (kind == DIAL_TASK_H1_WALK) {
              float zf = dm::fminf_(s.cdist[2 * f], s.cdist[2 * f + 1]);
              reward_gaits += (z_tar - zf) * (z_tar - zf);
              fz = zs;
            } else {
              float zf = dm::fminf_(dm::fminf_(s.cdist[4 * f], s.cdist[4 * f + 1]), dm::fminf_(s.cdist[4 * f + 2], s.cdist[4 * f + 3]));
              reward_gaits += (z_tar - zf) * (z_tar - zf);
              fz = zs;
            }
            if (FULL_INFO) {
              const bool contact = fz < 1e-3f;
              const bool filt = contact || (info[DIAL_INFO_LAST_CONTACT + f] != 0.f);
              info[DIAL_INFO_AIR_TIME + f] = (info[DIAL_INFO_AIR_TIME + f] + dt) * (filt ? 0.f : 1.f);
              info[DIAL_INFO_LAST_CONTACT + f] = contact ? 1.f : 0.f;
            }
          }
          out = -reward_gaits;
        } else {
          const int stage = (int)info[DIAL_INFO_STAGE];
          float reward_contact = 0.f, penalty_contact = 0.f;
          for (int i = 0; i < 4; i++) {
            bool pen = s.cdist[i] <= 0.001f;
            for (int j = 0; j < m->n_stage; j++) {
              float dx = s.cpos[3 * i] - tg->contact_targets[j][i][0], dy = s.cpos[3 * i + 1] - tg->contact_targets[j][i][1];
              bool cond = (dx * dx + dy * dy) <= tg->contact_radius[j][i] * tg->contact_radius[j][i];
              float val = (j == stage ? 1.f : 0.f) * dm::clip(s.cdist[i] * -1.0f + 1.0f, 0.f, 1.f);
              reward_contact += cond ? val : 0.f;
              pen = pen && !cond;
            }
            penalty_contact += pen ? 1.f : 0.f;
          }
          out = reward_contact;
          s.rpart[4] = penalty_contact;
        }
      } else if (it == 1) {
        float rot_u[4] = {uq[0], uq[1], uq[2], uq[3]};
        float up[3] = {0.f, 0.f, 1.f}, vec[3];
        dm::rotate(vec, up, rot_u);
        out = -((vec[0] - 0.f) * (vec[0] - 0.f) + (vec[1] - 0.f) * (vec[1] - 0.f) + (vec[2] - 1.f) * (vec[2] - 1.f));
      } else if (it == 2) {
        float rot_t[4] = {tq[0], tq[1], tq[2], tq[3]};
        const float yaw = quat_yaw(rot_t);
        if (walk) {
          float yaw_tar;
          if constexpr (PRE) yaw_tar = s.ztab[st * DIAL_ZTAB_W + DIAL_MAX_FEET + 3];
          else {
            const float a2 = cmd[5];
            const float avt = dm::fminf_(a2 * step * dt / m->ramp_up_time, a2);
            yaw_tar = yaw_tar0 + avt * dt * step;
          }
          const float d_yaw = yaw - yaw_tar;
          const float wy = d_yaw - 6.283185307179586f * DM_RINT(d_yaw * 0.15915494309189535f);
          out = -(wy * wy);
        } else {
          const float ey = yaw - tg->yaw_targets[(int)info[DIAL_INFO_STAGE]];
          out = -(ey * ey);
        }
      } else if (it == 3 || it == 4) {
        if (walk) {
          float rot_t[4] = {tq[0], tq[1], tq[2], tq[3]};
          float off[3] = {tp[0] - tcom[0], tp[1] - tcom[1], tp[2] - tcom[2]};
          float ang[3] = {tv[0], tv[1], tv[2]};
          if (it == 3) {
            float cr[3], vel[3], vb[3];
            dm::cross3(cr, off, ang);
            for (int k = 0; k < 3; k++) vel[k] = tv[3 + k] - cr[k];
            dm::inv_rotate(vb, vel, rot_t);
            float vt[2];
            for (int k = 0; k < 2; k++) {
              if constexpr (PRE) vt[k] = s.ztab[st * DIAL_ZTAB_W + DIAL_MAX_FEET + k];
              else { const float v = cmd[k]; vt[k] = dm::fminf_(v * step * dt / m->ramp_up_time, v); }
            }
            const float e0 = vb[0] - vt[0], e1 = vb[1] - vt[1];
            out = -(e0 * e0 + e1 * e1);
          } else {
            float ab[3], angs[3] = {ang[0] * DIAL_PI / 180.0f, ang[1] * DIAL_PI / 180.0f, ang[2] * DIAL_PI / 180.0f};
            dm::inv_rotate(ab, angs, rot_t);
            if (kind == DIAL_TASK_H1_LOCO) {
              float e3 = 0.f;
              for (int k = 0; k < 3; k++) {
                const float a = cmd[3 + k];
                const float e = ab[k] - dm::fminf_(a * step * dt / m->ramp_up_time, a);
                e3 += e * e;
              }
              out = -e3;
            } else {
              float avt;
              if constexpr (PRE) avt = s.ztab[st * DIAL_ZTAB_W + DIAL_MAX_FEET + 2];
              else { const float a2 = cmd[5]; avt = dm::fminf_(a2 * step * dt / m->ramp_up_time, a2); }
              const float ea = ab[2] - avt;
              out = -(ea * ea);
            }
          }
        } else if (it == 3) {
          const int stage = (int)info[DIAL_INFO_STAGE];
          float rp = 0.f;
          for (int k = 0; k < 3; k++) { float e = tp[k] - tg->pose_targets[stage][k]; rp += e * e; }
          out = -rp;
        } else {
          return s.rpart[4];
        }
      } else if (it == 5) {
        const float dh = tp[2] - pos_tar_z;
        out = -(dh * dh);
      } else if (it == 6) {
        float reward_energy = 0.f;
        if (kind == DIAL_TASK_H1_WALK || kind == DIAL_TASK_H1_PUSH_CRATE)
          for (int a = 0; a < nu; a++) { float e = s.ctrl[a] / m->tau_range[a][1]; reward_energy += e * e; }
        if (kind == DIAL_TASK_H1_LOCO) {
          for (int a = 0; a < nu; a++) { float e = s.ctrl[a] / m->tau_range[a][1] * s.qvel[6 + a] / 160.0f; reward_energy += e * e; }
          float lvl = 0.f;
          for (int f = 0; f < 2; f++) {
            const int si = m->feet_site[f], sb = m->site_bodyid[si];
            float bq[4] = {s.xquat[4 * sb], s.xquat[4 * sb + 1], s.xquat[4 * sb + 2], s.xquat[4 * sb + 3]};
            float sq[4] = {m->site_quat[si][0], m->site_quat[si][1], m->site_quat[si][2], m->site_quat[si][3]};
            float q[4], mat[9];
            dm::quat_mul(q, bq, sq);
            dm::quat_to_mat(mat, q);
            lvl += (mat[2] - 0.f) * (mat[2] - 0.f) + (mat[5] - 0.f) * (mat[5] - 0.f) + (mat[8] - 1.f) * (mat[8] - 1.f);
          }
          out = -reward_energy;
          s.rpart[8] = -lvl;
        } else {
          out = -reward_energy;
        }
      } else {
        float rot_t[4] = {tq[0], tq[1], tq[2], tq[3]};
        float up[3] = {0.f, 0.f, 1.f}, upv[3];
        dm::rotate(upv, up, rot_t);
        bool done = upv[2] < 0.f;
        for (int a = 0; a < nu; a++) {
          float q = s.qpos[7 + a];
          done = done || q < m->joint_range[a][0] || q > m->joint_range[a][1];
        }
        done = done || tp[2] < m->done_height;
        out = done ? 1.f : 0.f;
      }
      return out;
    };
    w.items(1 + (PRE ? dim_nq(m) : nu), [&](int it) {
      float* info = s.info;
      if (it > 0) {
        if (!walk && it <= nu) info[DIAL_INFO_LAST_CTRL + it - 1] = s.ctrl[it - 1];
        if constexpr (PRE) { if (w.out_io && w.out_io->qss) w.out_io->qss[(size_t)w.out_row * dim_nq(m) + (it - 1)] = s.qpos[it - 1]; }
        return;
      }
      float cmd[6] = {0.f, 0.f, 0.f, 0.f, 0.f, 0.f};
      if (walk && !PRE) step_cmd(m, tg, info[DIAL_INFO_STEP], cmd);
      float r[9];
      r[0] = term(std::integral_constant<int, 0>{}, cmd);
      r[1] = term(std::integral_constant<int, 1>{}, cmd);
      r[2] = term(std::integral_constant<int, 2>{}, cmd);
      r[3] = term(std::integral_constant<int, 3>{}, cmd);
      r[4] = term(std::integral_constant<int, 4>{}, cmd);
      r[5] = term(std::integral_constant<int, 5>{}, cmd);
      r[6] = term(std::integral_constant<int, 6>{}, cmd);
      r[7] = FULL_INFO ? term(std::integral_constant<int, 7>{}, cmd) : 0.f;
      r[8] = kind == DIAL_TASK_H1_LOCO ? s.rpart[8] : 0.f;
      if constexpr (kind == DIAL_TASK_H1_PUSH_CRATE) r[8] = pc_contact_reward(m, s);
      const float dt = m->dt, step = info[DIAL_INFO_STEP];
      float reward;
      if (kind == DIAL_TASK_GO2_WALK) {
        reward = r[0] * 0.1f + r[1] * 0.5f + r[2] * 0.3f + r[3] * 1.0f + r[4] * 1.0f + r[5] * 1.0f;
      } else if (kind == DIAL_TASK_H1_WALK) {
        reward = r[0] * 5.0f + r[1] * 0.5f + r[2] * 0.1f + r[3] * 1.0f + r[4] * 1.0f + r[5] * 0.5f + r[6] * 0.01f;
      } else if (kind == DIAL_TASK_H1_PUSH_CRATE) {
        reward = r[0] * 5.0f + r[1] * 0.01f + r[2] * 0.1f + r[3] * 1.0f + r[4] * 1.0f + r[5] * 0.5f + r[6] * 0.01f + r[8] * 0.05f;
      } else if (kind == DIAL_TASK_H1_LOCO) {
        reward = r[0] * 10.0f + r[1] * 0.5f + r[2] * 0.5f + r[3] * 1.0f + r[4] * 1.0f + r[5] * 0.5f +
                 r[8] * 0.02f + r[6] * 0.01f;
      } else {
        reward = r[3] * 1.0f + r[1] * 1.0f + r[2] * 0.3f + r[0] * 0.1f - r[4] * 0.1f + 1.0f * 10.0f;
      }
      if (walk && !PRE) {
        for (int k = 0; k < 3; k++) {
          const float v = cmd[k], a = cmd[3 + k];
          info[DIAL_INFO_VEL_TAR + k] = dm::fminf_(v * step * dt / m->ramp_up_time, v);
          info[DIAL_INFO_ANG_VEL_TAR + k] = dm::fminf_(a * step * dt / m->ramp_up_time, a);
        }
      }
      if (FULL_INFO) info[DIAL_INFO_DONE] = r[7];
      info[DIAL_INFO_STEP] = step + 1.f;
      if (kind == DIAL_TASK_GO2_SEQ_JUMP) {
        float st = DM_FLOOR(info[DIAL_INFO_STEP] * dt / m->jump_dt);
        info[DIAL_INFO_STAGE] = dm::fminf_(st, (float)(m->n_stage - 1));
      }
      info[DIAL_INFO_REWARD] = reward;
      if constexpr (PRE) { if (w.out_io && w.out_io->rewss) w.out_io->rewss[w.out_row] = reward; }
    });
  };
  {
    constexpr uint32_t kmask = task_kind_mask<typename M::D>();
    const int kind_u = DM_UNIFORM_I(m->kind);
    if ((kmask >> DIAL_TASK_GO2_WALK & 1u) && kind_u == DIAL_TASK_GO2_WALK) reward_phase(std::integral_constant<int, DIAL_TASK_GO2_WALK>{});
    else if ((kmask >> DIAL_TASK_GO2_SEQ_JUMP & 1u) && kind_u == DIAL_TASK_GO2_SEQ_JUMP) reward_phase(std::integral_constant<int, DIAL_TASK_GO2_SEQ_JUMP>{});
    else if ((kmask >> DIAL_TASK_H1_WALK & 1u) && kind_u == DIAL_TASK_H1_WALK) reward_phase(std::integral_constant<int, DIAL_TASK_H1_WALK>{});
    else if ((kmask >> DIAL_TASK_H1_LOCO & 1u) && kind_u == DIAL_TASK_H1_LOCO) reward_phase(std::integral_constant<int, DIAL_TASK_H1_LOCO>{});
    else if constexpr ((kmask >> DIAL_TASK_H1_PUSH_CRATE) & 1u) {
      if (kind_u == DIAL_TASK_H1_PUSH_CRATE) reward_phase(std::integral_constant<int, DIAL_TASK_H1_PUSH_CRATE>{});
    }
  }
  DIAL_MARK(w, 10);
  return s.info[DIAL_INFO_REWARD];
}

template <class W>
DIAL_DEV void init_world(W& w, const Ws& s) {
  w.items(1, [&](int) {
    for (int k = 0; k < 3; k++) { s.xpos[k] = 0.f; s.com[k] = 0.f; }
    s.xquat[0] = 1.f; s.xquat[1] = 0.f; s.xquat[2] = 0.f; s.xquat[3] = 0.f;
  });
}
template <class W, class M>
DIAL_DEV void init_square(W& w, const M* m, const Ws& s) {
  (void)m;
  if constexpr (M::D::square) w.items(M::D::NV * M::D::S, [&](int e) { s.M[e] = 0.f; });
  if constexpr (kQuadDims<typename M::D>) init_quad(w, m, s);
  if constexpr (W::half2) init_quad2(w, m, s);
  if constexpr (kQuadGenDims<typename M::D>) init_quad_gen(w, m, s);
}

}
```

### dial_mpc_amd/csrc/rollout_driver.h

```cpp
#pragma once
#include "rollout_body.h"
#include "philox.h"

namespace dial {


template <class W, class M>
DIAL_DEV void load_state(W& w, const M* m, const Ws& s, const float* state) {
  const int nq = dim_nq(m), nv = dim_nv(m);
  DIAL_LANE_SCOPE_IF(M::D::ell, w);
  w.items(nq + 2 * nv + DIAL_INFO_N, [&](int i) {
    float v = state[i];
    if (i < nq) s.qpos[i] = v;
    else if (i < nq + nv) s.qvel[i - nq] = v;
    else if (i < nq + 2 * nv) s.warm[i - nq - nv] = v;
    else s.info[i - nq - 2 * nv] = v;
  });
}
template <class W, class M>
DIAL_DEV void store_state(W& w, const M* m, const Ws& s, float* state) {
  const int nq = dim_nq(m), nv = dim_nv(m);
  DIAL_LANE_SCOPE_IF(M::D::ell, w);
  w.items(nq + 2 * nv + DIAL_INFO_N, [&](int i) {
    float v;
// ... 146 lines not shown
    trows = __builtin_amdgcn_readfirstlane(m->table_rows);
    if (trows > 0) {
      M* const c = const_cast<M*>(m);
      const int step = (int)s.info[DIAL_INFO_STEP], idx = table_row_index(step, m->table_row0, trows, m->table_mode);
      tnext = table_fetch(m, w.lane, idx, m->table_cols);
      if (w.lane == 0) { c->table_nidx = idx; c->table_nr = step + m->table_row0; }
      w.sync();
    }
  }
#endif
  if constexpr (PRE) {
    const bool walk = m->kind == DIAL_TASK_GO2_WALK || m->kind == DIAL_TASK_H1_WALK || m->kind == DIAL_TASK_H1_LOCO || m->kind == DIAL_TASK_H1_PUSH_CRATE;
    static_assert(DIAL_ZTAB_W == DIAL_MAX_FEET + 4, "ztab row: foot heights | v_x v_y yaw-rate yaw targets");
    if (walk) w.items((st_end - st_begin) * DIAL_ZTAB_W, [&](int it) {
      const int dt_ = it / DIAL_ZTAB_W, f = it - dt_ * DIAL_ZTAB_W;
      const float step = s.info[DIAL_INFO_STEP] + (float)dt_;
      float* row = s.ztab + (st_begin + dt_) * DIAL_ZTAB_W;
      if (f < DIAL_MAX_FEET) { if (f < m->nfeet) row[f] = gait_ztar(m, f, step); return; }
      float cmd[6];
      step_cmd(m, tg, step, cmd);
      const float dt = m->dt;
      if (f < DIAL_MAX_FEET + 2) { const float v = cmd[f - DIAL_MAX_FEET]; row[f] = dm::fminf_(v * step * dt / m->ramp_up_time, v); return; }
      const float a2 = cmd[5];
      const float avt = dm::fminf_(a2 * step * dt / m->ramp_up_time, a2);
      row[f] = f == DIAL_MAX_FEET + 2 ? avt : s.info[DIAL_INFO_YAW_TAR] + avt * dt * step;
    });
  }
  const auto packed = [&](int i) -> float* {
    const int off = i < nq ? i : (i < nq + nv ? (int)(s.qvel - s.qpos) + (i - nq)
                    : (i < nq + 2 * nv ? (int)(s.warm - s.qpos) + (i - nq - nv) : (int)(s.info - s.qpos) + (i - nq - 2 * nv)));
    return s.qpos + off;
  };
  bool mean_now = false;
  constexpr int KSTRIDE = W::half2 ? 32 : 64, NKEEP = W::half2 ? 4 : 2;
  float keep[NKEEP] = {};
  rsum_t msum = 0;
  (void)packed; (void)keep; (void)msum;
  for (int st_own = st_begin; mean_now || st_own < st_end;) {
    const int st = mean_now ? helper : st_own;
    const int row = mean_now ? io.n_noise : n;
    w.redraw_priority();
#ifndef DIAL_EMU
    if (w.launder) { asm volatile("" : "+v"(w.lane)); w.lane_r = w.lane; }
    if constexpr (M::D::user) {
      if (trows > 0 && !mean_now) {
        const int idx = m->table_nidx, cols = m->table_cols;
        table_publish(w, m, st & 1, idx, cols, tnext);
        if (st + 1 < st_end) {
          M* const c = const_cast<M*>(m);
          const int r = m->table_nr + 1, nidx = table_next_index(idx, r, trows, m->table_mode);
          tnext = table_fetch(m, w.lane, nidx, cols);
          w.sync();
          if (w.lane == 0) { c->table_nidx = nidx; c->table_nr = r; }
        }
      }
    }
#endif
    if constexpr (!PRE) {
      DIAL_LANE_SCOPE_IF(kRowsDims<typename M::D> && !M::D::gen, w);
      w.items(nu, [&](int a) {
        float u;
        if (mean_now && !io.us) {
          u = 0.f;
          for (int k = 0; k < Hn1; k++) u += cfg->W[st][k] * dm::clip(io.Ybar[k * nu + a], -1.f, 1.f);
        } else {
          u = node2u(st, a);
        }
        s.act[a] = u;
      });
    } else {
#ifndef DIAL_EMU
      if (mean_now) {
        w.items(nu, [&](int a) {
          float u = 0.f;
          for (int k = 0; k < Hn1; k++) u += cfg->W[st][k] * dm::clip(io.Ybar[k * nu + a], -1.f, 1.f);
          s.jtab[st * nu + a] = act2joint(m, u, a);
        });
      }
#endif
    }
    DIAL_MARK(w, 11);
    const int work0 = w.work;
    if constexpr (PRE) { w.out_io = &io; w.out_row = row * T + st; }
    float rew = env_step<false, PRE>(w, m, tg, s, st);
    if (mean_now) msum += (rsum_t)rew; else rsum += (rsum_t)rew;
#ifndef DIAL_EMU
    if constexpr (M::D::ell) {
      if (io.work_stat && relay < 0) {
        int lvl = 0;
        if (w.lane == 0) {
          const int tot_w = atomicAdd(io.work_stat, w.work - work0) + (w.work - work0);
          const int tot_s = atomicAdd(io.work_stat + 1, 1) + 1;
          const float own = (float)w.work * (float)tot_s, avg = (float)tot_w * (float)(st + 1 - st_begin);
#ifndef DIAL_LAG_T1
#define DIAL_LAG_T1 1.0f
#define DIAL_LAG_T2 1.2f
#define DIAL_LAG_T3 1.4f
#endif
          lvl = own > DIAL_LAG_T3 * avg ? 3 : (own > DIAL_LAG_T2 * avg ? 2 : (own > DIAL_LAG_T1 * avg ? 1 : 0));
        }
        w.prio_level = __builtin_amdgcn_readfirstlane(lvl);
      }
    }
#endif
    const size_t o = (size_t)row * T + st;
    if constexpr (!PRE) {
      float* const qrow = io.qss ? io.qss + o * nq : nullptr;
      float* const qdrow = io.qdss ? io.qdss + o * nv : nullptr;
      float* const xrow = io.xss ? io.xss + o * nx : nullptr;
      float* const rrow = io.rewss ? io.rewss + o : nullptr;
      const int nmax = nx > nq ? nx : nq;
      w.items(nmax, [&](int i) {
        if (qrow && i < nq) qrow[i] = s.qpos[i];
        if (qdrow && i < nv) qdrow[i] = s.qvel[i];
        if (xrow && i < nx) xrow[i] = s.xpos[3 + i];
        if (rrow && i == 0) rrow[0] = rew;
      });
    }
    (void)o;
#ifndef DIAL_PROFILE
    if constexpr (TRACE) { if (io.trace) store_state(w, m, s, io.trace + o * nstate); }
#endif
    DIAL_MARK(w, 24);
#ifndef DIAL_EMU
    if (mean_now) {
      if (helper + 1 < T) {
        store_state(w, m, s, io.relay_buf);
        w.items(1, [&](int) { store_sum(io.relay_buf + nstate, msum); });
        __builtin_amdgcn_fence(__ATOMIC_RELEASE, "agent");
        if (w.lane == 0) __hip_atomic_store(io.relay_flag, helper + 1, __ATOMIC_RELEASE, __HIP_MEMORY_SCOPE_AGENT);
      } else {
        if (io.rews) { const float mean = (float)(msum / (rsum_t)T); w.items(1, [&](int) { io.rews[row] = mean; }); }
        if (w.lane == 0) __hip_atomic_store(io.relay_flag, 0, __ATOMIC_RELEASE, __HIP_MEMORY_SCOPE_AGENT);
      }
      w.items(KSTRIDE, [&](int l) {
#pragma unroll
        for (int k = 0; k < NKEEP; k++) if (l + k * KSTRIDE < nstate) *packed(l + k * KSTRIDE) = keep[k];
      });
      mean_now = false;
      continue;
    }
#endif
    st_own++;
#ifndef DIAL_EMU
    if (helper >= 0 && st == helper && relay < 0) {
#pragma unroll
      for (int k = 0; k < NKEEP; k++) keep[k] = w.lane + k * KSTRIDE < nstate ? *packed(w.lane + k * KSTRIDE) : 0.f;
      w.sync();
      bool ok = true;
      if (helper == 0) {
        load_state(w, m, s, io.state);
        msum = 0;
        if (io.Y0s) {
          DIAL_LANE_SCOPE(w);
          w.items(Hn1 * nu, [&](int it) { io.Y0s[(size_t)io.n_noise * Hn1 * nu + it] = dm::clip(io.Ybar[it], -1.f, 1.f); });
        }
      } else {
        int timed_out = 0;
        if (w.lane == 0) {
          unsigned spins = 0;
          while (__hip_atomic_load(io.relay_flag, __ATOMIC_ACQUIRE, __HIP_MEMORY_SCOPE_AGENT) != helper && ++spins < (1u << 20))
            __builtin_amdgcn_s_sleep(2);
          timed_out = spins >= (1u << 20);
        }
        timed_out = __builtin_amdgcn_readfirstlane(timed_out);
        if (timed_out) {
          if (w.lane == 0) {
            if (io.err_word) __hip_atomic_store(io.err_word, 1, __ATOMIC_RELEASE, __HIP_MEMORY_SCOPE_SYSTEM);
            if (io.rews) reinterpret_cast<uint32_t*>(io.rews)[io.n_noise] = 0x7fc00000u;
          }
          ok = false;
        } else {
          __builtin_amdgcn_wave_barrier();
          __builtin_amdgcn_fence(__ATOMIC_ACQUIRE, "agent");
          load_state(w, m, s, io.relay_buf);
          msum = load_sum(io.relay_buf + nstate);
        }
      }
      mean_now = ok;
    }
#endif
  }
#ifdef DIAL_PROFILE
  DIAL_MARK(w, 11);
  if (io.prof && n == 0 && w.lane == 0) for (int k = 0; k < 28; k++) io.prof[k] = w.acc[k];
  if (io.prof && w.lane == 0) for (int k = 28; k < DIAL_NSEC; k++) atomicAdd(&io.prof[k], w.acc[k]);
#endif
#ifndef DIAL_EMU
  if (relay >= 0 && relay + 1 == io.debug_stall_piece1) return;
  if (relay >= 0 && st_end < T) {
    store_state(w, m, s, rbuf);
    w.items(1, [&](int) { store_sum(rbuf + nstate, rsum); });
    __builtin_amdgcn_fence(__ATOMIC_RELEASE, "agent");
    if (w.lane == 0) __hip_atomic_store(rflag, relay + 1, __ATOMIC_RELEASE, __HIP_MEMORY_SCOPE_AGENT);
    return;
  }
  if (relay >= 0 && w.lane == 0) __hip_atomic_store(rflag, 0, __ATOMIC_RELEASE, __HIP_MEMORY_SCOPE_AGENT);
#endif
  if (io.rews) {
    const float mean = (float)(rsum / (rsum_t)T);
    w.items(1, [&](int) { io.rews[n] = mean; });
  }
}

template <class W, class M>
DIAL_DEV void env_step_single(W& w, const M* m, const dial_task* tg, const Ws& s, float* state,
                              const float* action, float* xpos_out, float* xquat_out, float* ctrl_out) {
  init_world(w, s);
  init_square(w, m, s);
  load_state(w, m, s, state);
  w.items(dim_nu(m), [&](int a) { s.act[a] = action[a]; });
  env_step<true>(w, m, tg, s);
  store_state(w, m, s, state);
  const int nb1 = dim_nb(m) - 1;
  w.items(nb1 * 7 + dim_nu(m), [&](int i) {
    if (i < nb1 * 3) { if (xpos_out) xpos_out[i] = s.xpos[3 + i]; }
    else if (i < nb1 * 7) { if (xquat_out) xquat_out[i - nb1 * 3] = s.xquat[4 + (i - nb1 * 3)]; }
    else { if (ctrl_out) ctrl_out[i - nb1 * 7] = s.ctrl[i - nb1 * 7]; }
  });
}

template <class W, class M>
DIAL_DEV void env_reset_single(W& w, const M* m, const Ws& s, const float* qpos, const float* qvel, float* state,
                               float* xpos_out, float* xquat_out) {
  init_world(w, s);
  init_square(w, m, s);
  const int nq = dim_nq(m), nv = dim_nv(m);
  w.items(nq + 2 * nv + DIAL_INFO_N + dim_nu(m), [&](int i) {
    if (i < nq) s.qpos[i] = qpos[i];
    else if (i < nq + nv) s.qvel[i - nq] = qvel[i - nq];
    else if (i < nq + 2 * nv) s.warm[i - nq - nv] = 0.f;
    else if (i < nq + 2 * nv + DIAL_INFO_N) {
      const int k = i - nq - 2 * nv;
      s.info[k] = (k >= DIAL_INFO_POS_TAR && k < DIAL_INFO_POS_TAR + 3) ? m->init_pos_tar[k - DIAL_INFO_POS_TAR]
                  : ((k >= DIAL_INFO_ANG_VEL_TAR && k < DIAL_INFO_ANG_VEL_TAR + 3) ? m->init_ang_vel_tar[k - DIAL_INFO_ANG_VEL_TAR] : 0.f);
    } else s.ctrl[i - nq - 2 * nv - DIAL_INFO_N] = 0.f;
  });
  forward(w, m, s);
  store_state(w, m, s, state);
  const int nb1 = dim_nb(m) - 1;
  w.items(nb1 * 7, [&](int i) {
    if (i < nb1 * 3) { if (xpos_out) xpos_out[i] = s.xpos[3 + i]; }
    else { if (xquat_out) xquat_out[i - nb1 * 3] = s.xquat[4 + (i - nb1 * 3)]; }
  });
}

}
```

### dial_mpc_amd/csrc/smooth_quad.h

```cpp
#pragma once
#include "derived.h"
#include "dmath.h"

#ifndef DIAL_NO_SITE_SHORTCUT
#define DIAL_NO_SITE_SHORTCUT 0
#endif

namespace dial {

template <class D>
inline constexpr bool kQuadDims = D::quad_stage;
template <class D>
inline constexpr bool kQuadGenDims = D::quad_gen;

template <bool FUSED = true, class W, class M>
DIAL_DEV void forward_smooth_quad(W& w, const M* m, const Ws& s) {
  constexpr int S = M::D::S;
  static_assert(M::D::NB >= 14 && M::D::NV == 18, "quadruped layout: trunk + 4 legs of 3");
  static_assert(!FUSED || (M::D::NB == 14 && M::D::NC == 4 && M::D::square), "fused foot contacts: the Go2's own scene");
  static_assert(FUSED || !M::D::square, "generic feature set: packed M");
  DIAL_MARK(w, 15);
#if !defined(DIAL_EMU) && !defined(DIAL_QUAD_HOIST)
  const int lane_keep = w.lane;
  { int lq = w.lane; asm volatile("" : "+v"(lq)); w.lane = lq; }
// ... 126 lines not shown
      const float jp[3] = {m->jnt_pos[ji][0], m->jnt_pos[ji][1], m->jnt_pos[ji][2]};
      const float ja[3] = {m->jnt_axis[ji][0], m->jnt_axis[ji][1], m->jnt_axis[ji][2]};
      float anchor[3], jaxis[3], cr[3];
      if (m->body_flags[b] & 2) { anchor[0] = 0.f; anchor[1] = 0.f; anchor[2] = 0.f; }
      else dm::rotate(anchor, jp, bq);
      for (int k = 0; k < 3; k++) anchor[k] += lane_val(PL[k], l);
      dm::rotate(jaxis, ja, bq);
      const float offj[3] = {com[0] - anchor[0], com[1] - anchor[1], com[2] - anchor[2]};
      dm::cross3(cr, jaxis, offj);
      const float w0 = kd == 3 ? 1.f : 0.f, w1 = kd == 4 ? 1.f : 0.f, w2 = kd == 5 ? 1.f : 0.f;
      for (int k = 0; k < 3; k++) {
        const float ta = w0 * cdT[0][k] + w1 * cdT[1][k] + w2 * cdT[2][k];
        const float tl = (k == kd ? 1.f : 0.f) + (w0 * cdT[0][3 + k] + w1 * cdT[1][3 + k] + w2 * cdT[2][3 + k]);
        o[10 + k] = leg ? jaxis[k] : (tdof ? ta : 0.f);
        o[13 + k] = leg ? cr[k] : (tdof ? tl : 0.f);
      }
    });
    DIAL_UNROLL_FULL
    for (int k = 0; k < 10; k++) X[k] = T[k];
    DIAL_UNROLL_FULL
    for (int k = 0; k < 6; k++) CD[k] = T[10 + k];
  }
  DIAL_MARK(w, 18);
  vfloat VA[12];
  {
    const float qv[6] = {s.qvel[0], s.qvel[1], s.qvel[2], s.qvel[3], s.qvel[4], s.qvel[5]};
    const float vs[6] = {0.f, 0.f, 0.f, qv[0], qv[1], qv[2]};
    float velT[6] = {0.f, 0.f, 0.f, qv[0], qv[1], qv[2]};
    float accT[6] = {0.f, 0.f, 0.f, -m->gravity[0], -m->gravity[1], -m->gravity[2]};
    for (int j = 0; j < 3; j++) {
      float cl[3];
      dm::cross3(cl, vs + 3, cdT[j]);
      for (int k = 0; k < 3; k++) accT[3 + k] += cl[k] * qv[3 + j];
      for (int k = 0; k < 6; k++) velT[k] += cdT[j][k] * qv[3 + j];
    }
    w.per_lane_n(VA, [&](int l, float* o) {
      for (int k = 0; k < 6; k++) { o[k] = velT[k]; o[6 + k] = accT[k]; }
    });
  }
  const vfloat QVL = w.per_lane([&](int l) {
    const int d = l & 15, r = l >> 4;
    const bool leg = d >= 1 && d <= 3, tdof = r == 0 && d >= 4 && d <= 9;
    return s.qvel[leg ? 3 * r + d + 5 : (tdof ? d - 4 : 0)];
  });
  {
    const vfloat QL = w.per_lane([&](int l) { const int d = l & 15; return (d >= 1 && d <= 3) ? lane_val(QVL, l) : 0.f; });
    const auto chain_sum = [&](vfloat* acc, const vfloat* cd) {
      vfloat P[6], P1[6], P2[6];
      DIAL_UNROLL_FULL
      for (int k = 0; k < 6; k++) P[k] = cd[k] * QL;
      DIAL_UNROLL_FULL
      for (int k = 0; k < 6; k++) { P2[k] = w.template row_shr<2>(P[k]); P1[k] = w.template row_shr<1>(P[k]); }
      DIAL_UNROLL_FULL
      for (int k = 0; k < 6; k++) acc[k] = vfma(cd[k], QL, (acc[k] + P2[k]) + P1[k]);
    };
    chain_sum(VA, CD);
    vfloat VP[6], CDD[6];
    DIAL_UNROLL_FULL
    for (int k = 0; k < 6; k++) VP[k] = w.template row_shr<1>(VA[k]);
    w.per_lane_n(CDD, [&](int l, float* o) {
      const float vp[6] = {lane_val(VP[0], l), lane_val(VP[1], l), lane_val(VP[2], l), lane_val(VP[3], l), lane_val(VP[4], l), lane_val(VP[5], l)};
      const float cd[6] = {lane_val(CD[0], l), lane_val(CD[1], l), lane_val(CD[2], l), lane_val(CD[3], l), lane_val(CD[4], l), lane_val(CD[5], l)};
      dm::motion_cross(o, vp, cd);
    });
    chain_sum(VA + 6, CDD);
  }
  float* xrow = nullptr;
  if constexpr (M::D::pre_ctrl) { if (w.out_io && w.out_io->xss) xrow = w.out_io->xss + (size_t)w.out_row * ((M::D::NB - 1) * 3); }
  w.items(64, [&](int l) {
    const int d = l & 15, r = l >> 4;
    const bool leg = d >= 1 && d <= 3;
    const int b = leg ? 3 * r + d + 1 : 1;
    if (leg || l == 0) {
      for (int k = 0; k < 3; k++) s.xpos[3 * b + k] = lane_val(PL[k], l);
      if constexpr (M::D::pre_ctrl) { if (xrow) for (int k = 0; k < 3; k++) xrow[3 * (b - 1) + k] = lane_val(PL[k], l); }
      store4(s.xquat + 4 * b, lane_val(PL[3], l), lane_val(PL[4], l), lane_val(PL[5], l), lane_val(PL[6], l));
      for (int k = 0; k < 3; k++) store2(s.cvel + 6 * b + 2 * k, lane_val(VA[2 * k], l), lane_val(VA[2 * k + 1], l));
    }
    if (l == 0) {
      for (int k = 0; k < 3; k++) { s.com[3 * m->body_rootid[1] + k] = com[k]; s.spos[k] = lane_val(F[16 + k], l); }
      for (int k = 0; k < 4; k++) s.qpos[3 + k] = tquat[k];
    }
    if (d == 3) for (int k = 0; k < 3; k++) s.spos[3 * (1 + r) + k] = lane_val(F[16 + k], l);
    if constexpr (!FUSED) {
      for (int e = l; e < M::D::NTRI; e += 64) s.M[e] = 0.f;
    }
  });
  if constexpr (FUSED) {
    const float pn[3] = {m->geom0_normal[0], m->geom0_normal[1], m->geom0_normal[2]};
    const float fr[9] = {s.cframe[0], s.cframe[1], s.cframe[2], s.cframe[3], s.cframe[4], s.cframe[5], s.cframe[6], s.cframe[7], s.cframe[8]};
    vfloat CP[4];
    w.per_lane_n(CP, [&](int l, float* o) {
      const int r = l >> 4, g2 = 1 + r;
      const float ctr[3] = {lane_val(F[19], l), lane_val(F[20], l), lane_val(F[21], l)};
      const float radius = m->geom_size[g2][0];
      const float diff[3] = {ctr[0] - m->geom_pos[0][0], ctr[1] - m->geom_pos[0][1], ctr[2] - m->geom_pos[0][2]};
      const float dist = dm::dot3(diff, pn) - radius;
      for (int k = 0; k < 3; k++) o[k] = ctr[k] - pn[k] * (radius + 0.5f * dist);
      o[3] = dist;
    });
    vfloat PC[3];
    DIAL_UNROLL_FULL
    for (int k = 0; k < 3; k++) PC[k] = w.template row_bcast<3>(CP[k]);
    w.items(64, [&](int l) {
      const int d = l & 15, r = l >> 4;
      const bool leg = d >= 1 && d <= 3, tk = d >= 4 && d <= 9;
      if (!(leg || tk)) return;
      const int i = leg ? 3 * r + d + 5 : d - 4;
      const float mu1 = m->con_friction[r][0], mu2 = m->con_friction[r][1];
      const float cd[6] = {lane_val(CD[0], l), lane_val(CD[1], l), lane_val(CD[2], l), lane_val(CD[3], l), lane_val(CD[4], l), lane_val(CD[5], l)};
      const float off[3] = {lane_val(PC[0], l) - com[0], lane_val(PC[1], l) - com[1], lane_val(PC[2], l) - com[2]};
      float cr[3];
      dm::cross3(cr, cd, off);
      const float diff[3] = {cd[3] + cr[0], cd[4] + cr[1], cd[5] + cr[2]};
      const float jn = dm::dot3(fr, diff), t1 = dm::dot3(fr + 3, diff) * mu1, t2 = dm::dot3(fr + 6, diff) * mu2;
      store4(s.Jc + i * M::D::T + 4 * r, jn + t1, jn - t1, jn + t2, jn - t2);
    });
    w.items(64, [&](int l) {
      const int d = l & 15, r = l >> 4;
      if (d != 3) return;
      const float mu1 = m->con_friction[r][0], mu2 = m->con_friction[r][1];
      const float pos = lane_val(CP[3], l) - m->con_margin[r];
      const float invweight = m->con_invw[r][0];
      float k_, b_, imp;
      kbi(m->kbi_tab[m->con_kbi[r]], pos, k_, b_, imp);
      const float Rr = dm::fmaxf_(invweight * (1.f - imp) / imp, MJ_MINVAL);
      const float va[3] = {lane_val(VA[0], l), lane_val(VA[1], l), lane_val(VA[2], l)};
      const float off[3] = {lane_val(CP[0], l) - com[0], lane_val(CP[1], l) - com[1], lane_val(CP[2], l) - com[2]};
      float cr[3];
      dm::cross3(cr, va, off);
      const float vp[3] = {lane_val(VA[3], l) + cr[0], lane_val(VA[4], l) + cr[1], lane_val(VA[5], l) + cr[2]};
      const float vn = dm::dot3(fr, vp), v1 = dm::dot3(fr + 3, vp) * mu1, v2 = dm::dot3(fr + 6, vp) * mu2;
      const bool on = pos < 0.f;
      const float dd = on ? 1.f / Rr : 0.f, ar = -k_ * imp * pos;
      constexpr int NL = M::D::NL;
      store4(s.D + NL + 4 * r, dd, dd, dd, dd);
      store4(s.aref + NL + 4 * r, on ? ar - b_ * (vn + v1) : 0.f, on ? ar - b_ * (vn - v1) : 0.f, on ? ar - b_ * (vn + v2) : 0.f, on ? ar - b_ * (vn - v2) : 0.f);
      s.cdist[r] = lane_val(CP[3], l);
      for (int k = 0; k < 3; k++) s.cpos[3 * r + k] = lane_val(CP[k], l);
    });
    w.items(64, [&](int l) {
      const int d = l & 15, r = l >> 4;
      if (!(d >= 1 && d <= 3)) return;
      const int b = 3 * r + d + 1, ji = b - 1, i = b + 4, qa = b + 5, lr = m->dof_limrow[i];
      if (lr < 0) return;
      const float q = s.qpos[qa];
      const float dist_min = q - m->jnt_range[ji][0], dist_max = m->jnt_range[ji][1] - q;
      const float pos = dm::fminf_(dist_min, dist_max) - m->jnt_margin[ji];
      const float sgn = dist_min < dist_max ? 1.f : -1.f;
      float k_, b_, imp;
      kbi(m->kbi_tab[m->jnt_kbi[ji]], pos, k_, b_, imp);
      const float Rr = dm::fmaxf_(m->dof_invweight0[i] * (1.f - imp) / imp, MJ_MINVAL);
      const bool on = pos < 0.f;
      s.lsign[lr] = sgn;
      s.D[lr] = on ? 1.f / Rr : 0.f;
      s.aref[lr] = on ? -b_ * (sgn * lane_val(QVL, l)) - k_ * imp * pos : 0.f;
    });
  }
  DIAL_MARK(w, 19);
  {
    vfloat T[6];
    w.per_lane_n(T, [&](int l, float* o) {
      const bool body = (l & 15) <= 3;
      float ci[10], ca[6], cv[6], f1[6], f2[6], f3[6];
      for (int k = 0; k < 10; k++) ci[k] = lane_val(X[k], l);
      for (int k = 0; k < 6; k++) { cv[k] = lane_val(VA[k], l); ca[k] = lane_val(VA[6 + k], l); }
// ... 159 lines not shown
```

### dial_mpc_amd/csrc/wave.h

```cpp
#pragma once
#include "rollout_io.h"

#ifdef DIAL_EMU
#include <cmath>
#include <cstdio>
#include <cstring>
#include <vector>
#define DIAL_DEV inline
#define DIAL_UNROLL


struct vbool { bool x[64]; };
struct vfloat {
  float x[64];
};
inline vfloat vsplat(float v) { vfloat r; for (int l = 0; l < 64; l++) r.x[l] = v; return r; }
inline vfloat operator+(const vfloat& a, const vfloat& b) { vfloat r; for (int l = 0; l < 64; l++) r.x[l] = a.x[l] + b.x[l]; return r; }
inline vfloat operator-(const vfloat& a, const vfloat& b) { vfloat r; for (int l = 0; l < 64; l++) r.x[l] = a.x[l] - b.x[l]; return r; }
inline vfloat operator*(const vfloat& a, const vfloat& b) { vfloat r; for (int l = 0; l < 64; l++) r.x[l] = a.x[l] * b.x[l]; return r; }
inline vfloat operator*(const vfloat& a, float b) { vfloat r; for (int l = 0; l < 64; l++) r.x[l] = a.x[l] * b; return r; }
inline vfloat vfma(const vfloat& a, const vfloat& b, const vfloat& c) { vfloat r; for (int l = 0; l < 64; l++) r.x[l] = std::fma(a.x[l], b.x[l], c.x[l]); return r; }
inline vfloat vsel(const vbool& c, const vfloat& a, const vfloat& b) { vfloat r; for (int l = 0; l < 64; l++) r.x[l] = c.x[l] ? a.x[l] : b.x[l]; return r; }
inline vbool vlt0(const vfloat& a) { vbool r; for (int l = 0; l < 64; l++) r.x[l] = a.x[l] < 0.f; return r; }
inline vbool veq0(const vfloat& a) { vbool r; for (int l = 0; l < 64; l++) r.x[l] = a.x[l] == 0.f; return r; }
inline float bcast(const vfloat& v, int lane) { return v.x[lane]; }
inline float lane_val(const vfloat& v, int lane) { return v.x[lane]; }
inline void load2(const float* p, float& a, float& b) { a = p[0]; b = p[1]; }
inline void load4(const float* p, float& a, float& b, float& c, float& d) { a = p[0]; b = p[1]; c = p[2]; d = p[3]; }
inline void store2(float* p, float a, float b) { p[0] = a; p[1] = b; }
inline void store4(float* p, float a, float b, float c, float d) { p[0] = a; p[1] = b; p[2] = c; p[3] = d; }
inline float fast_rsqrt(float x) { return 1.0f / std::sqrt(x); }
inline float fast_rcp(float x) { return 1.0f / x; }
inline vfloat vrcp(const vfloat& a) { vfloat r; for (int l = 0; l < 64; l++) r.x[l] = 1.0f / a.x[l]; return r; }

inline float emu_row_tree(const float* v) {
  float s1[16], s2[16], s3[16];
  for (int l = 0; l < 16; l++) s1[l] = v[l] + v[l ^ 1];
  for (int l = 0; l < 16; l++) s2[l] = s1[l] + s1[l ^ 2];
  for (int l = 0; l < 16; l++) s3[l] = s2[l] + s2[(l & 8) | (7 - (l & 7))];
  return s3[15] + s3[0];
}
inline float emu_tree64(const float* v) {
  const float r0 = emu_row_tree(v), r1 = emu_row_tree(v + 16), r2 = emu_row_tree(v + 32), r3 = emu_row_tree(v + 48);
  return (r3 + r2) + (r1 + r0);
}
inline float emu_tree32(const float* v) {
  return emu_row_tree(v) + emu_row_tree(v + 16);
}

#define DIAL_MARK(w, id)
#define DIAL_LANE_SCOPE(w)
#define DIAL_LANE_SCOPE_IF(cond, w)
struct Wave {
  static constexpr bool half2 = false;
  bool tree_sums = false;
  bool launder = false;
  const dial::RolloutIO* out_io = nullptr;
  int out_row = 0;
  const float* jrow = nullptr;
  float* lds = nullptr;
  int lds_words = 0;
  bool check_races = false;
  int races = 0;
  int phase = 0;

  bool nancheck = false, nan_seen = false;
  void scan_nonfinite() {
    if (!nancheck || nan_seen) return;
    for (int k = 0; k < lds_words; k++)
      if (!std::isfinite(lds[k])) {
        std::fprintf(stderr, "[wave_emu] first non-finite LDS word after phase #%d: word %d = %g\n", phase, k, (double)lds[k]);
        nan_seen = true;
        return;
      }
  }
  template <class F>
  void items(int count, F f) {
    phase++;
    if (!check_races) {
      for (int i = 0; i < count; i++) f(i);
      scan_nonfinite();
      return;
    }
    std::vector<float> snap(lds, lds + lds_words);
    for (int i = 0; i < count; i++) f(i);
    std::vector<float> fwd(lds, lds + lds_words);
    std::memcpy(lds, snap.data(), sizeof(float) * lds_words);
    for (int i = count - 1; i >= 0; i--) f(i);
    if (std::memcmp(fwd.data(), lds, sizeof(float) * lds_words) != 0) {
      if (races < 10) {
        int w = 0;
        for (; w < lds_words; w++)
          if (std::memcmp(&fwd[w], &lds[w], 4) != 0) break;
        std::fprintf(stderr, "[wave_emu] intra-phase dependence in phase #%d (first differing LDS word %d)\n", phase, w);
      }
      races++;
    }
  }
  template <class F>
  float sum(int count, F f) {
    if (tree_sums) {
      float v[64];
      for (int l = 0; l < 64; l++) { v[l] = l < count ? f(l) : 0.f; for (int i = l + 64; i < count; i += 64) v[l] += f(i); }
      return emu_tree64(v);
    }
    float s = 0.f;
    for (int i = 0; i < count; i++) s += f(i);
    return s;
  }
  template <class F>
  void sum3(int count, F f, float& a, float& b, float& c) {
    if (tree_sums) {
      float va[64], vb[64], vc[64];
      for (int l = 0; l < 64; l++) {
        va[l] = vb[l] = vc[l] = 0.f;
        if (l < count) f(l, va[l], vb[l], vc[l]);
        for (int i = l + 64; i < count; i += 64) { float x = 0.f, y = 0.f, z = 0.f; f(i, x, y, z); va[l] += x; vb[l] += y; vc[l] += z; }
      }
      a = emu_tree64(va); b = emu_tree64(vb); c = emu_tree64(vc);
      return;
    }
    a = b = c = 0.f;
    for (int i = 0; i < count; i++) {
      float x = 0.f, y = 0.f, z = 0.f;
      f(i, x, y, z);
      a += x; b += y; c += z;
    }
  }
  template <class F>
  float maxv(int count, F f) {
    float s = -INFINITY;
    for (int i = 0; i < count; i++) { float v = f(i); s = v > s ? v : s; }
    return s;
  }
  template <class F>
  vfloat per_lane(F f) { vfloat r; for (int l = 0; l < 64; l++) r.x[l] = f(l); return r; }
  template <class F>
// ... 4 lines not shown
  }
  vfloat quad_xor1(const vfloat& v) { vfloat r; for (int l = 0; l < 64; l++) r.x[l] = v.x[l ^ 1]; return r; }
  vfloat quad_xor2(const vfloat& v) { vfloat r; for (int l = 0; l < 64; l++) r.x[l] = v.x[l ^ 2]; return r; }
  template <class F>
  void per_lane4(F f, vfloat& a, vfloat& b, vfloat& c, vfloat& d) {
    for (int l = 0; l < 64; l++) { const float* p = f(l); a.x[l] = p[0]; b.x[l] = p[1]; c.x[l] = p[2]; d.x[l] = p[3]; }
  }
  template <class F>
  void per_lane4_r(F f, vfloat& a, vfloat& b, vfloat& c, vfloat& d) { per_lane4(f, a, b, c, d); }
  template <int N>
  vfloat row_shr(const vfloat& v) { vfloat r; for (int l = 0; l < 64; l++) r.x[l] = (l & 15) >= N ? v.x[l - N] : 0.f; return r; }
  template <int N>
  vfloat row_shl(const vfloat& v) { vfloat r; for (int l = 0; l < 64; l++) r.x[l] = (l & 15) + N <= 15 ? v.x[l + N] : 0.f; return r; }
  template <int N>
  vfloat row_shr_lo(const vfloat& v) { vfloat r; for (int l = 0; l < 64; l++) r.x[l] = ((l & 15) < 8 && (l & 15) >= N) ? v.x[l - N] : 0.f; return r; }
  template <int N>
  vfloat row_shl_lo(const vfloat& v) { vfloat r; for (int l = 0; l < 64; l++) r.x[l] = (l & 15) < 8 ? v.x[l + N] : 0.f; return r; }
  template <int N>
  vfloat row_bcast(const vfloat& v) { vfloat r; for (int l = 0; l < 64; l++) r.x[l] = v.x[(l & ~15) + N]; return r; }
  unsigned long long mask(const vbool& c) const { unsigned long long b = 0; for (int l = 0; l < 64; l++) b |= (unsigned long long)(c.x[l] ? 1 : 0) << l; return b; }
  vbool lane_gt(int k) const { vbool r; for (int l = 0; l < 64; l++) r.x[l] = l > k; return r; }
  vbool lane_eq(int k) const { vbool r; for (int l = 0; l < 64; l++) r.x[l] = l == k; return r; }
  vbool lane_lt(int k) const { vbool r; for (int l = 0; l < 64; l++) r.x[l] = l < k; return r; }
  void begin_region() {}
  void set_rollout(int) {}
  void redraw_priority() {}
  int work = 0;
  vfloat lane_reverse(const vfloat& v, int n) { vfloat r; for (int l = 0; l < 64; l++) r.x[l] = l < n ? v.x[n - 1 - l] : 0.f; return r; }
  void fence() {}
  vfloat row16_sum(const vfloat& v) {
    vfloat r;
    for (int g = 0; g < 4; g++) {
      float t = 0.f;
      for (int l = 0; l < 16; l++) t += v.x[16 * g + l];
      for (int l = 0; l < 16; l++) r.x[16 * g + l] = t;
    }
    return r;
  }
  void row16_sum3(vfloat& a, vfloat& b, vfloat& c) { a = row16_sum(a); b = row16_sum(b); c = row16_sum(c); }
  template <class F>
  int compact(int count, F pred, float* list) {
    int n = 0;
    for (int l = 0; l < count && l < 64; l++) if (pred(l)) list[n++] = (float)l;
    return n;
  }
  template <int K>
  void row16_sumN(vfloat (&v)[K]) { for (int k = 0; k < K; k++) v[k] = row16_sum(v[k]); }
  template <int K>
  void seg8_sumN(vfloat (&v)[K]) {
    for (int k = 0; k < K; k++) {
      vfloat s1, s2, s3;
      for (int l = 0; l < 64; l++) s1.x[l] = v[k].x[l] + v[k].x[l ^ 1];
      for (int l = 0; l < 64; l++) s2.x[l] = s1.x[l] + s1.x[l ^ 2];
      for (int l = 0; l < 64; l++) s3.x[l] = s2.x[l] + s2.x[(l & ~7) | (7 - (l & 7))];
      v[k] = s3;
    }
  }
  template <class F>
  vfloat gather64(const vfloat& v, F src) { vfloat r; for (int l = 0; l < 64; l++) r.x[l] = v.x[src(l) & 63]; return r; }
  float vsum(const vfloat& v) { if (tree_sums) return emu_tree64(v.x); float s = 0.f; for (int l = 0; l < 64; l++) s += v.x[l]; return s; }
  template <int K>
  void vsumN(vfloat (&v)[K], float (&out)[K]) { for (int k = 0; k < K; k++) out[k] = vsum(v[k]); }
  template <int K>
  float bc(const vfloat& v) { return v.x[K]; }
  void dup_rows(const vfloat& v, vfloat& X, vfloat& Y) {
    for (int l = 0; l < 64; l++) { X.x[l] = v.x[(l & 32) | (l & 15)]; Y.x[l] = v.x[(l & 32) | 16 | (l & 15)]; }
  }
  void dup_halves(const vfloat& v, vfloat& LO, vfloat& HI) {
    for (int l = 0; l < 64; l++) { LO.x[l] = v.x[l & 31]; HI.x[l] = v.x[32 | (l & 31)]; }
  }
  template <int K>
  float rowbc(const vfloat& v) { return v.x[K]; }
  template <int K>
  vfloat mul_pick(const vfloat& X, const vfloat& Y, const vfloat& other) { return other * pick<K>(X, Y); }
  template <int K>
  vfloat pick(const vfloat& X, const vfloat& Y) { if constexpr (K < 16) return row_bcast<K>(X); else return row_bcast<K - 16>(Y); }
  template <int K>
  vfloat fma_pick(const vfloat& acc, const vfloat& X, const vfloat& Y, const vfloat& other) { return acc + other * pick<K>(X, Y); }
  template <int K>
  vfloat fnma_pick(const vfloat& acc, const vfloat& X, const vfloat& Y, const vfloat& other) { return acc - other * pick<K>(X, Y); }
  template <int K>
  vfloat rcp_pick(const vfloat& X, const vfloat& Y) { return vrcp(pick<K>(X, Y)); }
};

struct WaveH : Wave {
  static constexpr bool half2 = true;
  template <class F>
  float sum(int count, F f) {
    float v[32];
    for (int l = 0; l < 32; l++) { v[l] = l < count ? f(l) : 0.f; for (int i = l + 32; i < count; i += 32) v[l] += f(i); }
    return emu_tree32(v);
  }
  template <class F>
  void sum3(int count, F f, float& a, float& b, float& c) {
    float va[32], vb[32], vc[32];
    for (int l = 0; l < 32; l++) {
      va[l] = vb[l] = vc[l] = 0.f;
      if (l < count) f(l, va[l], vb[l], vc[l]);
      for (int i = l + 32; i < count; i += 32) { float x = 0.f, y = 0.f, z = 0.f; f(i, x, y, z); va[l] += x; vb[l] += y; vc[l] += z; }
    }
    a = emu_tree32(va); b = emu_tree32(vb); c = emu_tree32(vc);
  }
  template <class F>
  vfloat per_lane(F f) { vfloat r; for (int l = 0; l < 64; l++) r.x[l] = f(l & 31); return r; }
  template <class F>
  vfloat per_lane_r(F f) { return per_lane(f); }
  template <int K, class F>
  void per_lane_n(vfloat (&out)[K], F f) {
    for (int l = 0; l < 64; l++) { float o[K]; f(l & 31, o); for (int k = 0; k < K; k++) out[k].x[l] = o[k]; }
  }
  template <class F>
  void per_lane4(F f, vfloat& a, vfloat& b, vfloat& c, vfloat& d) {
    for (int l = 0; l < 64; l++) { const float* p = f(l & 31); a.x[l] = p[0]; b.x[l] = p[1]; c.x[l] = p[2]; d.x[l] = p[3]; }
  }
  unsigned long long mask(const vbool& c) const { unsigned long long b = 0; for (int l = 0; l < 32; l++) b |= (unsigned long long)(c.x[l] ? 1 : 0) << l; return b; }
  vbool lane_gt(int k) const { vbool r; for (int l = 0; l < 64; l++) r.x[l] = (l & 31) > k; return r; }
  vbool lane_eq(int k) const { vbool r; for (int l = 0; l < 64; l++) r.x[l] = (l & 31) == k; return r; }
  vbool lane_lt(int k) const { vbool r; for (int l = 0; l < 64; l++) r.x[l] = (l & 31) < k; return r; }
  vfloat lane_reverse(const vfloat& v, int n) { vfloat r; for (int l = 0; l < 64; l++) r.x[l] = (l & 31) < n ? v.x[(l & 32) + n - 1 - (l & 31)] : 0.f; return r; }
  float vsum(const vfloat& v) { return emu_tree32(v.x); }
  template <int K>
  void vsumN(vfloat (&v)[K], float (&out)[K]) { for (int k = 0; k < K; k++) out[k] = vsum(v[k]); }
  template <class F>
  vfloat gather(const vfloat& v, F src) { vfloat r; for (int l = 0; l < 64; l++) r.x[l] = v.x[(l & 32) | (src(l & 31) & 31)]; return r; }
  vfloat grp8_bcast3(const vfloat& v) { vfloat r; for (int l = 0; l < 64; l++) r.x[l] = v.x[(l & ~7) | 3]; return r; }
};

#else
#include <hip/hip_runtime.h>
#define DIAL_DEV __device__ __forceinline__

namespace dialwave {
template <int CTRL, int ROW_MASK = 0xf, int BANK_MASK = 0xf, bool BOUND = true>
__device__ __forceinline__ float dpp_add(float v) {
  int moved = __builtin_amdgcn_update_dpp(0, __builtin_bit_cast(int, v), CTRL, ROW_MASK, BANK_MASK, BOUND);
  return v + __builtin_bit_cast(float, moved);
}
__device__ __forceinline__ float wave_sum_dpp(float v) {
  v = dpp_add<0xb1>(v);
  v = dpp_add<0x4e>(v);
  v = dpp_add<0x141>(v);
  v = dpp_add<0x140>(v);
  v = dpp_add<0x142, 0xa>(v);
  v = dpp_add<0x143, 0xc>(v);
  return __builtin_bit_cast(float, __builtin_amdgcn_readlane(__builtin_bit_cast(int, v), 63));
}
__device__ __forceinline__ float wave_sum_shfl(float v) {
  for (int o = 32; o > 0; o >>= 1) v += __shfl_xor(v, o, 64);
  return __builtin_bit_cast(float, __builtin_amdgcn_readfirstlane(__builtin_bit_cast(int, v)));
}
__device__ __forceinline__ float wave_max_shfl(float v) {
  for (int o = 32; o > 0; o >>= 1) { float t = __shfl_xor(v, o, 64); v = t > v ? t : v; }
  return __builtin_bit_cast(float, __builtin_amdgcn_readfirstlane(__builtin_bit_cast(int, v)));
}
#ifdef DIAL_NO_DPP
__device__ __forceinline__ float wave_sum(float v) { return wave_sum_shfl(v); }
#else
__device__ __forceinline__ float wave_sum(float v) { return wave_sum_dpp(v); }
#endif
}


using vfloat = float;
using vbool = bool;
__device__ __forceinline__ vfloat vsplat(float v) { return v; }
__device__ __forceinline__ vfloat vfma(vfloat a, vfloat b, vfloat c) { return __builtin_fmaf(a, b, c); }
__device__ __forceinline__ vfloat vsel(vbool c, vfloat a, vfloat b) { return c ? a : b; }
__device__ __forceinline__ vbool vlt0(vfloat a) { return a < 0.f; }
__device__ __forceinline__ vbool veq0(vfloat a) { return a == 0.f; }
__device__ __forceinline__ float bcast(vfloat v, int lane) {
  return __builtin_bit_cast(float, __builtin_amdgcn_readlane(__builtin_bit_cast(int, v), lane));
}
__device__ __forceinline__ float lane_val(vfloat v, int) { return v; }
__device__ __forceinline__ void load2(const float* p, float& a, float& b) { const float2 t = *reinterpret_cast<const float2*>(p); a = t.x; b = t.y; }
__device__ __forceinline__ void load4(const float* p, float& a, float& b, float& c, float& d) { const float4 t = *reinterpret_cast<const float4*>(p); a = t.x; b = t.y; c = t.z; d = t.w; }
__device__ __forceinline__ void store2(float* p, float a, float b) { *reinterpret_cast<float2*>(p) = make_float2(a, b); }
__device__ __forceinline__ void store4(float* p, float a, float b, float c, float d) { *reinterpret_cast<float4*>(p) = make_float4(a, b, c, d); }
__device__ __forceinline__ float fast_rsqrt(float x) { return __builtin_amdgcn_rsqf(x); }
__device__ __forceinline__ float fast_rcp(float x) { return __builtin_amdgcn_rcpf(x); }
__device__ __forceinline__ vfloat vrcp(vfloat a) { return __builtin_amdgcn_rcpf(a); }

template <class W>
struct LaneScope {
  W& w;
  int keep, keep_r;
  __device__ __forceinline__ explicit LaneScope(W& w_) : w(w_), keep(w_.lane), keep_r(w_.lane_r) {
    int lq = w.lane;
    asm volatile("" : "+v"(lq));
    w.lane = lq;
    w.lane_r = lq;
  }
  __device__ __forceinline__ ~LaneScope() { w.lane = keep; w.lane_r = keep_r; }
};
#define DIAL_LANE_SCOPE(w) LaneScope<std::remove_reference_t<decltype(w)>> dial_lane_scope_(w)
template <bool COND, class W>
struct LaneScopeIf {
  __device__ __forceinline__ explicit LaneScopeIf(W&) {}
};
template <class W>
struct LaneScopeIf<true, W> : LaneScope<W> {
  __device__ __forceinline__ explicit LaneScopeIf(W& w_) : LaneScope<W>(w_) {}
};
#define DIAL_LANE_SCOPE_IF(cond, w) LaneScopeIf<(cond), std::remove_reference_t<decltype(w)>> dial_lane_scope_if_(w)
#ifdef DIAL_PROFILE
#define DIAL_NSEC 32
#define DIAL_MARK(w, id) (w).mark(id)
#elif defined(DIAL_ISA_MARKS)
#define DIAL_MARK(w, id) asm volatile("; DIAL_MARK %0" ::"n"(id))
#else
#define DIAL_MARK(w, id)
#endif
struct Wave {
  static constexpr bool half2 = false;
  int lane;
  const dial::RolloutIO* out_io = nullptr;
  int out_row = 0;
  const float* jrow = nullptr;
#ifdef DIAL_PROFILE
  unsigned long long tprev = 0;
  unsigned long long* acc = nullptr;
  __device__ __forceinline__ void mark(int id) {
    unsigned long long t = __builtin_readcyclecounter();
    if (lane == 0 && acc) acc[id] += t - tprev;
    tprev = t;
  }
#endif
  __device__ __forceinline__ void sync() {
#ifdef DIAL_BLOCK_SYNC
    __syncthreads();
#else
    __builtin_amdgcn_fence(__ATOMIC_RELEASE, "wavefront");
    __builtin_amdgcn_wave_barrier();
    __builtin_amdgcn_fence(__ATOMIC_ACQUIRE, "wavefront");
#endif
  }

  template <class F>
  __device__ __forceinline__ void items(int count, F f) {
    for (int i = lane; i < count; i += 64) f(i);
    sync();
  }
  template <class F>
  __device__ __forceinline__ float sum(int count, F f) {
    float v = lane < count ? f(lane) : 0.f;
    for (int i = lane + 64; i < count; i += 64) v += f(i);
    return dialwave::wave_sum(v);
  }
  template <class F>
  __device__ __forceinline__ void sum3(int count, F f, float& a, float& b, float& c) {
    float x = 0.f, y = 0.f, z = 0.f;
    if (lane < count) f(lane, x, y, z);
    for (int i = lane + 64; i < count; i += 64) {
      float x2 = 0.f, y2 = 0.f, z2 = 0.f;
      f(i, x2, y2, z2);
      x += x2; y += y2; z += z2;
    }
    vfloat t3[3] = {x, y, z};
    float r3[3];
    vsumN(t3, r3);
    a = r3[0]; b = r3[1]; c = r3[2];
  }
  template <class F>
  __device__ __forceinline__ float maxv(int count, F f) {
    float v = lane < count ? f(lane) : -INFINITY;
    for (int i = lane + 64; i < count; i += 64) { const float u = f(i); v = u > v ? u : v; }
    return dialwave::wave_max_shfl(v);
  }
  template <class F>
  __device__ __forceinline__ vfloat per_lane(F f) { return f(lane); }
  template <class F>
  __device__ __forceinline__ vfloat per_lane_r(F f) { return f(lane_r); }
  template <int K, class F>
  __device__ __forceinline__ void per_lane_n(vfloat (&out)[K], F f) {
    float o[K];
    f(lane, o);
#pragma unroll
    for (int k = 0; k < K; k++) out[k] = o[k];
  }
  __device__ __forceinline__ vfloat quad_xor1(vfloat v) {
    return __builtin_bit_cast(float, __builtin_amdgcn_update_dpp(0, __builtin_bit_cast(int, v), 0xb1, 0xf, 0xf, true));
  }
  __device__ __forceinline__ vfloat quad_xor2(vfloat v) {
    return __builtin_bit_cast(float, __builtin_amdgcn_update_dpp(0, __builtin_bit_cast(int, v), 0x4e, 0xf, 0xf, true));
  }
  template <int N>
  __device__ __forceinline__ vfloat row_shr(vfloat v) {
    return __builtin_bit_cast(float, __builtin_amdgcn_update_dpp(0, __builtin_bit_cast(int, v), 0x110 + N, 0xf, 0xf, true));
  }
  template <int N>
  __device__ __forceinline__ vfloat row_shl(vfloat v) {
    return __builtin_bit_cast(float, __builtin_amdgcn_update_dpp(0, __builtin_bit_cast(int, v), 0x100 + N, 0xf, 0xf, true));
  }
  template <int N>
  __device__ __forceinline__ vfloat row_shr_lo(vfloat v) {
    return __builtin_bit_cast(float, __builtin_amdgcn_update_dpp(0, __builtin_bit_cast(int, v), 0x110 + N, 0xf, 0x3, true));
  }
// ... 90 lines not shown
#pragma unroll
    for (int k = 0; k < K; k++) v[k] = dialwave::dpp_add<0xb1>(v[k]);
#pragma unroll
    for (int k = 0; k < K; k++) v[k] = dialwave::dpp_add<0x4e>(v[k]);
#pragma unroll
    for (int k = 0; k < K; k++) v[k] = dialwave::dpp_add<0x141>(v[k]);
#pragma unroll
    for (int k = 0; k < K; k++) v[k] = dialwave::dpp_add<0x140>(v[k]);
  }
  template <int K>
  __device__ __forceinline__ void seg8_sumN(vfloat (&v)[K]) {
#pragma unroll
    for (int k = 0; k < K; k++) v[k] = dialwave::dpp_add<0xb1>(v[k]);
#pragma unroll
    for (int k = 0; k < K; k++) v[k] = dialwave::dpp_add<0x4e>(v[k]);
#pragma unroll
    for (int k = 0; k < K; k++) v[k] = dialwave::dpp_add<0x141>(v[k]);
  }
  template <class F>
  __device__ __forceinline__ vfloat gather64(vfloat v, F src) { return __shfl(v, src(lane) & 63, 64); }
  __device__ __forceinline__ void row16_sum3(vfloat& a, vfloat& b, vfloat& c) {
    a = dialwave::dpp_add<0xb1>(a); b = dialwave::dpp_add<0xb1>(b); c = dialwave::dpp_add<0xb1>(c);
    a = dialwave::dpp_add<0x4e>(a); b = dialwave::dpp_add<0x4e>(b); c = dialwave::dpp_add<0x4e>(c);
    a = dialwave::dpp_add<0x141>(a); b = dialwave::dpp_add<0x141>(b); c = dialwave::dpp_add<0x141>(c);
    a = dialwave::dpp_add<0x140>(a); b = dialwave::dpp_add<0x140>(b); c = dialwave::dpp_add<0x140>(c);
  }
  template <int K>
  __device__ __forceinline__ float bc(vfloat v) { return bcast(v, K); }
  __device__ __forceinline__ void dup_rows(vfloat v, vfloat& X, vfloat& Y) {
    const auto r = __builtin_amdgcn_permlane16_swap(__builtin_bit_cast(unsigned, v), __builtin_bit_cast(unsigned, v), false, false);
    const unsigned r0 = r[0], r1 = r[1];
    X = __builtin_bit_cast(float, r0);
    Y = __builtin_bit_cast(float, r1);
#ifdef DIAL_FUSED_DPP
    asm("s_nop 1" : "+v"(X), "+v"(Y));
#endif
  }
  __device__ __forceinline__ void dup_halves(vfloat v, vfloat& LO, vfloat& HI) {
    const auto r = __builtin_amdgcn_permlane32_swap(__builtin_bit_cast(unsigned, v), __builtin_bit_cast(unsigned, v), false, false);
    const unsigned r0 = r[0], r1 = r[1];
    LO = __builtin_bit_cast(float, r0);
    HI = __builtin_bit_cast(float, r1);
  }
  template <int K>
  __device__ __forceinline__ float rowbc(vfloat v) { return row_bcast<K>(v); }
  template <int K>
  __device__ __forceinline__ vfloat pick(vfloat X, vfloat Y) { if constexpr (K < 16) return row_bcast<K>(X); else return row_bcast<K - 16>(Y); }
#ifdef DIAL_FUSED_DPP
#define DIAL_DPP_TAIL " row_newbcast:%3 row_mask:0xf bank_mask:0xf bound_ctrl:1"
  template <int K>
  __device__ __forceinline__ vfloat fma_pick(vfloat acc, vfloat X, vfloat Y, vfloat other) {
    asm("v_fmac_f32_dpp %0, %1, %2" DIAL_DPP_TAIL : "+v"(acc) : "v"(K < 16 ? X : Y), "v"(other), "n"(K & 15));
    return acc;
  }
  template <int K>
  __device__ __forceinline__ vfloat fnma_pick(vfloat acc, vfloat X, vfloat Y, vfloat other) {
    asm("v_fmac_f32_dpp %0, -%1, %2" DIAL_DPP_TAIL : "+v"(acc) : "v"(K < 16 ? X : Y), "v"(other), "n"(K & 15));
    return acc;
  }
  template <int K>
  __device__ __forceinline__ vfloat rcp_pick(vfloat X, vfloat Y) {
    vfloat r;
    asm("v_rcp_f32_dpp %0, %1 row_newbcast:%2 row_mask:0xf bank_mask:0xf bound_ctrl:1" : "=v"(r) : "v"(K < 16 ? X : Y), "n"(K & 15));
    return r;
  }
  template <int K>
  __device__ __forceinline__ vfloat mul_pick(vfloat X, vfloat Y, vfloat other) {
    vfloat r;
    asm("v_mul_f32_dpp %0, %1, %2" DIAL_DPP_TAIL : "=v"(r) : "v"(K < 16 ? X : Y), "v"(other), "n"(K & 15));
    return r;
  }
#undef DIAL_DPP_TAIL
#else
  template <int K>
  __device__ __forceinline__ vfloat mul_pick(vfloat X, vfloat Y, vfloat other) { return other * pick<K>(X, Y); }
  template <int K>
  __device__ __forceinline__ vfloat fma_pick(vfloat acc, vfloat X, vfloat Y, vfloat other) { return acc + other * pick<K>(X, Y); }
  template <int K>
  __device__ __forceinline__ vfloat fnma_pick(vfloat acc, vfloat X, vfloat Y, vfloat other) { return acc - other * pick<K>(X, Y); }
  template <int K>
  __device__ __forceinline__ vfloat rcp_pick(vfloat X, vfloat Y) { return vrcp(pick<K>(X, Y)); }
#endif
};

struct WaveH : Wave {
  static constexpr bool half2 = true;
  int half;
  __device__ __forceinline__ void init(int tid) { lane = tid & 31; lane_r = lane; half = (tid >> 5) & 1; }
  template <class F>
  __device__ __forceinline__ void items(int count, F f) {
    for (int i = lane; i < count; i += 32) f(i);
    sync();
  }
  static __device__ __forceinline__ float half_combine(float v) {
    const auto r = __builtin_amdgcn_permlane16_swap(__builtin_bit_cast(unsigned, v), __builtin_bit_cast(unsigned, v), false, false);
    const unsigned r0 = r[0], r1 = r[1];
    return __builtin_bit_cast(float, r0) + __builtin_bit_cast(float, r1);
  }
  template <int K>
  __device__ __forceinline__ float bc(vfloat v) {
    static_assert(K >= 0 && K < 32, "logical lane");
    vfloat X, Y;
    dup_rows(v, X, Y);
    if constexpr (K < 16) return row_bcast<K>(X);
    else return row_bcast<K - 16>(Y);
  }
  template <class F>
  __device__ __forceinline__ vfloat gather(vfloat v, F src) { return __shfl(v, (src(lane) & 31) + 32 * half, 64); }
  __device__ __forceinline__ vfloat grp8_bcast3(vfloat v) {
    const vfloat a = row_bcast<3>(v), b = row_bcast<11>(v);
    return (lane & 8) ? b : a;
  }

  static __device__ __forceinline__ float opaque(float v) { asm("" : "+v"(v)); return v; }
  __device__ __forceinline__ vfloat row16_sum(vfloat v) { return Wave::row16_sum(opaque(v)); }
  template <int K>
  __device__ __forceinline__ void row16_sumN(vfloat (&v)[K]) {
#pragma unroll
    for (int k = 0; k < K; k++) v[k] = opaque(v[k]);
    Wave::row16_sumN(v);
  }
  __device__ __forceinline__ void row16_sum3(vfloat& a, vfloat& b, vfloat& c) { a = opaque(a); b = opaque(b); c = opaque(c); Wave::row16_sum3(a, b, c); }
  __device__ __forceinline__ float vsum(vfloat v) { return half_combine(row16_sum(v)); }
  template <int K>
  __device__ __forceinline__ void vsumN(vfloat (&v)[K], float (&out)[K]) {
    row16_sumN(v);
#pragma unroll
    for (int k = 0; k < K; k++) out[k] = half_combine(v[k]);
  }
  template <class F>
  __device__ __forceinline__ float sum(int count, F f) {
    float v = lane < count ? f(lane) : 0.f;
    for (int i = lane + 32; i < count; i += 32) v += f(i);
    return vsum(v);
  }
  template <class F>
  __device__ __forceinline__ void sum3(int count, F f, float& a, float& b, float& c) {
    float x = 0.f, y = 0.f, z = 0.f;
    if (lane < count) f(lane, x, y, z);
    for (int i = lane + 32; i < count; i += 32) {
      float x2 = 0.f, y2 = 0.f, z2 = 0.f;
      f(i, x2, y2, z2);
      x += x2; y += y2; z += z2;
    }
    vfloat t3[3] = {x, y, z};
    float r3[3];
    vsumN(t3, r3);
    a = r3[0]; b = r3[1]; c = r3[2];
  }
  __device__ __forceinline__ unsigned long long mask(vbool c) const {
    const unsigned long long b = __builtin_amdgcn_ballot_w64(c);
    return half ? (unsigned)(b >> 32) : (unsigned)b;
  }
  __device__ __forceinline__ vfloat lane_reverse(vfloat v, int n) {
    const float r = __shfl(v, ((n - 1 - lane) & 31) + 32 * half, 64);
    return lane < n ? r : 0.f;
  }
  __device__ __forceinline__ void set_rollout(int n) { const bool held = prio_held; Wave::set_rollout(__builtin_amdgcn_readfirstlane(n)); prio_held = held; }
  __device__ __forceinline__ void redraw_priority() {
#ifndef DIAL_FIXED_PRIORITY
    if (prio_held) return;
    prio_ctr++;
    const unsigned h = __builtin_amdgcn_readfirstlane((prio_seed + prio_ctr * 0x9E3779B1u) >> 30);
    if (h == 0) __builtin_amdgcn_s_setprio(0);
    else if (h == 1) __builtin_amdgcn_s_setprio(1);
    else if (h == 2) __builtin_amdgcn_s_setprio(2);
// ... 13 lines not shown
```

### include/dial_mpc.h

```cpp
#ifndef DIAL_MPC_H
#define DIAL_MPC_H

#include <stdint.h>
#include <stddef.h>

#ifdef __cplusplus
extern "C" {
#endif

#define DIAL_MAX_BODY 24
#define DIAL_MAX_JNT 24
#define DIAL_MAX_Q 32
#define DIAL_MAX_V 28
#define DIAL_MAX_U 20
#define DIAL_MAX_GEOM 20
#define DIAL_MAX_SITE 8
#define DIAL_MAX_CON 56
#define DIAL_MAX_EFC 240
#define DIAL_MAX_LIM 24
#define DIAL_MAX_FRI 4
#define DIAL_MAX_FEET 4
#define DIAL_MAX_STAGE 12
#define DIAL_MAX_T 36
#define DIAL_MAX_NODE 10
// ... 159 lines not shown
  int32_t act_dofadr[DIAL_MAX_U];
  int32_t act_qposadr[DIAL_MAX_U];
  int32_t act_ctrllimited[DIAL_MAX_U];
  int32_t act_isposition[DIAL_MAX_U];
  float act_gear[DIAL_MAX_U];
  float act_kp[DIAL_MAX_U];
  float act_ctrlrange[DIAL_MAX_U][2];
} dial_model;

typedef struct dial_task {
  int32_t kind;
  int32_t n_frames;
  int32_t position_control;
  int32_t torso_x;
  int32_t upright_x;
  int32_t nfeet;
  int32_t feet_site[DIAL_MAX_FEET];
  int32_t n_stage;
  float dt;
  float action_scale;
  float kp[DIAL_MAX_U];
  float kd[DIAL_MAX_U];
  float joint_range[DIAL_MAX_U][2];
  float phys_range[DIAL_MAX_U][2];
  float tau_range[DIAL_MAX_U][2];
  float foot_radius;
  float gait_duty;
  float gait_cadence;
  float gait_amp;
  float gait_phase[DIAL_MAX_FEET];
  float cmd_vel[3];
  float cmd_ang_vel[3];
  float ramp_up_time;
  float done_height;
  float jump_dt;
  float contact_targets[DIAL_MAX_STAGE][4][3];
  float contact_radius[DIAL_MAX_STAGE][4];
  float pose_targets[DIAL_MAX_STAGE][3];
  float yaw_targets[DIAL_MAX_STAGE];
  float init_pos_tar[3];
  float init_ang_vel_tar[3];
  float joint_offset[DIAL_MAX_U];
  int32_t randomize_tasks;
  int32_t n_cmd;
  float cmd_table[DIAL_MAX_CMD][3];
  int32_t crate_contact[DIAL_MAX_FEET];
  float crate_region[6];
  float head_vec[3];
  int32_t pc_foot_contact[2][2];
  int32_t pc_wanted[2];
  int32_t pc_n_unwanted;
  int32_t pc_unwanted[16];
  float pc_wanted_zmax;
} dial_task;

typedef struct dial_cfg {
  int32_t Nsample;
  int32_t Hsample;
  int32_t Hnode;
  float temp_sample;
  float W[DIAL_MAX_T][DIAL_MAX_NODE];
  float V[DIAL_MAX_NODE][DIAL_MAX_T];
} dial_cfg;

static inline int dial_state_size(int nq, int nv) { return nq + 2 * nv + DIAL_INFO_N; }

typedef struct dial_ctx dial_ctx;

typedef struct dial_options {
  int32_t force_generic;
  int32_t con_cap;
  int32_t no_queue;
  int32_t no_relay;
  int32_t relay_always;
  int32_t relay_steps;
  int32_t no_split_mask;
  int32_t debug_relay_stall;
  int32_t no_slice;
  int32_t slice_steps;
  int32_t no_lag_priority;
  int32_t no_mean_inline;
  int32_t no_spread;
  int32_t pair_mode;
  int32_t plan_cap;
} dial_options;

int dial_create(dial_ctx** out, const dial_model* model, const dial_task* task,
                const dial_cfg* cfg, int device);
int dial_create_sharded(dial_ctx** out, const dial_model* model, const dial_task* task,
                        const dial_cfg* cfg, int device, int n_local_cap);
int dial_create_ex(dial_ctx** out, const dial_model* model, const dial_task* task, const dial_cfg* cfg, int device,
                   int n_local_cap, const dial_options* opts);
void dial_destroy(dial_ctx* ctx);
const char* dial_last_error(const dial_ctx* ctx);

int dial_rollout(dial_ctx* ctx, const float* state, const float* us, int B, float* rewss,
                 float* qss, float* qdss, float* xposs, void* stream);

int dial_reverse_once(dial_ctx* ctx, const float* state, const float* Ybar_in,
                      const float* noise_scale, int ns, const float* eps, float* Ybar_out,
                      float* rews, float* qbar, float* qdbar, float* xbar, void* stream);

#define DIAL_SHARD_LEAN 2
int dial_shard_rollout(dial_ctx* ctx, const float* state, const float* Ybar_in,
                       const float* noise_scale, int ns, const float* eps, int n_local,
                       int with_mean, float* rews_local, void* stream);
int dial_shard_reduce(dial_ctx* ctx, const float* rews_all, int n_total, int n_begin,
                      int n_local, int with_mean, float* packed_out, void* stream);
int dial_shard_ybar(dial_ctx* ctx, const float* rews_all, int n_total, const float* eps_all,
                    const float* Ybar_in, const float* noise_scale, int ns, float* Ybar_out, void* stream);

int dial_reverse_once_rng(dial_ctx* ctx, const float* state, const float* Ybar_in, const float* noise_scale,
                          int ns, uint64_t seed, uint32_t counter, float* Ybar_out, float* rews, float* qbar,
                          float* qdbar, float* xbar, void* stream);
int dial_shard_rollout_rng(dial_ctx* ctx, const float* state, const float* Ybar_in, const float* noise_scale,
                           int ns, uint64_t seed, uint32_t counter, int n_begin, int n_local, int with_mean,
                           float* rews_local, void* stream);
int dial_rng_fill(dial_ctx* ctx, uint64_t seed, uint32_t counter, int n_begin, int n_count, float* eps_out,
                  void* stream);
int dial_shard_ybar_rng(dial_ctx* ctx, const float* rews_all, int n_total, uint64_t seed, uint32_t counter,
                        const float* Ybar_in, const float* noise_scale, int ns, float* Ybar_out, void* stream);
int dial_shard_pack_rewards(dial_ctx* ctx, const float* gathered, int world, int per, int n_total,
                            float* rews_all, void* stream);
int dial_shard_ybar_gathered(dial_ctx* ctx, const float* gathered, int world, int per, int n_total, const float* eps_all,
                             const float* Ybar_in, const float* noise_scale, int ns, float* rews_all_out, float* Ybar_out,
                             void* stream);
int dial_shard_ybar_gathered_rng(dial_ctx* ctx, const float* gathered, int world, int per, int n_total, uint64_t seed,
                                 uint32_t counter, const float* Ybar_in, const float* noise_scale, int ns,
                                 float* rews_all_out, float* Ybar_out, void* stream);
int dial_shard_reduce_gathered(dial_ctx* ctx, const float* gathered, int world, int per, int n_total, int n_begin,
                               int n_local, int with_mean, float* rews_all_out, float* packed_out, void* stream);

int dial_reverse_once_batch(dial_ctx* ctx, const float* states, const float* Ybar_in, const float* noise_scale, int ns,
                            const float* eps, int M, float* Ybar_out, float* rews, float* qbar, float* qdbar, float* xbar,
                            void* stream);
int dial_reverse_once_batch_rng(dial_ctx* ctx, const float* states, const float* Ybar_in, const float* noise_scale, int ns,
                                uint64_t seed, uint32_t counter, int M, float* Ybar_out, float* rews, float* qbar, float* qdbar,
                                float* xbar, void* stream);

int dial_shift(dial_ctx* ctx, float* Y, void* stream);
int dial_shift_batch(dial_ctx* ctx, float* Y, int M, void* stream);

int dial_env_step(dial_ctx* ctx, float* state, const float* action, float* xpos_out,
                  float* xquat_out, float* ctrl_out, void* stream);
int dial_env_step_batch(dial_ctx* ctx, float* states, const float* actions, float* xpos_out,
                        float* xquat_out, float* ctrl_out, int M, void* stream);

int dial_env_reset(dial_ctx* ctx, const float* qpos, const float* qvel, float* state,
                   float* xpos_out, float* xquat_out, void* stream);
int dial_env_reset_batch(dial_ctx* ctx, const float* qpos, const float* qvel, float* states,
                         float* xpos_out, float* xquat_out, int n, void* stream);

int dial_set_timing(dial_ctx* ctx, int enable);
int dial_get_rollout_ms(dial_ctx* ctx, double* total_ms, int* launches);

int dial_status(dial_ctx* ctx);

int dial_set_state_trace(dial_ctx* ctx, float* trace, int rows);

int dial_create_plugin(dial_ctx** out, const dial_model* model, const dial_task* task, const dial_cfg* cfg, int device,
                       const dial_options* opts, const char* plugin_path, const float* params, int n_params);
int dial_set_user_params(dial_ctx* ctx, const float* params, int n);
int dial_set_plan_params(dial_ctx* ctx, const float* params, int rows);
int dial_user_control(dial_ctx* ctx, const float* states, const float* actions, int n, float* ctrl_out, void* stream);
int dial_set_user_table(dial_ctx* ctx, const float* table, int rows, int cols, int row0, int mode);

// ... 16 lines not shown
```

Measured before the change: 5.915 million.

## Defer Go2 per-step reward computation to a batched epilogue over stashed state

Adds a deferred-reward rollout kernel for Go2 walking. During each step it stashes the torso pose, COM, velocity and foot heights into LDS, skips the per-step reward phase, and computes all rewards in one parallel epilogue across the horizon. This takes the serial reward work off each step's critical path and spreads it over lanes. In exchange it uses extra LDS per block, which can lower occupancy, and the kernel is loaded from a separate library through dlopen. The dial_options struct gains a field, which changes the ABI.

After: 6.039 million, median of 6. 2.1% higher.

```diff
diff --git a/dial_mpc_amd/_lib.py b/dial_mpc_amd/_lib.py
--- a/dial_mpc_amd/_lib.py
+++ b/dial_mpc_amd/_lib.py
@@ -37,7 +37,9 @@
         build_plant_var(force=force, verbose=verbose)
         build_plan_var(force=force, verbose=verbose)
         build_plan_ens(force=force, verbose=verbose)
+        build_reward_defer(force=force, verbose=verbose)
     return _build_lib(IEEE_LIB_PATH if ieee else LIB_PATH, [(os.path.join(_CSRC, "dial_hip.hip"), [], "dial_hip.o")] +
+                      ([(os.path.join(_CSRC, "reward_defer.hip"), [], "reward_defer.o")] if ieee else []) +
                       [(os.path.join(_CSRC, "kern_family.hip"), [f"-DDIAL_FAMILY={k}"] + _FAMILY_FLAGS.get(k, []), f"kern_family_{k}.o")
                        for k in range(N_FAMILIES)], force, verbose, ieee)
 
@@ -73,6 +75,13 @@
 def build_plan_var(force: bool = False, verbose: bool = False) -> str:
     return _build_lib(PLAN_VAR_LIB_PATH, [(os.path.join(_CSRC, "plan_var_family.hip"), [f"-DDIAL_FAMILY={k}"] + _FAMILY_FLAGS.get(k, []),
                                            f"plan_var_family_{k}.o") for k in range(N_PLANT_FAMILIES)], force, verbose, False)
+
+
+REWARD_DEFER_LIB_PATH = os.path.join(_CSRC, "libdialdefer.so")
+
+
+def build_reward_defer(force: bool = False, verbose: bool = False) -> str:
+    return _build_lib(REWARD_DEFER_LIB_PATH, [(os.path.join(_CSRC, "reward_defer.hip"), [], "reward_defer.o")], force, verbose, False)
 
 
 PLAN_ENS_LIB_PATH = os.path.join(_CSRC, "libdialplanens.so")
@@ -809,7 +818,8 @@
         self._check(self.lib.dial_set_state_trace(self.h, _ptr(self._trace), int(rows)), "dial_set_state_trace")
         return self._trace
 
-    LAUNCH_FIELDS = ("inst", "wpb", "blocks", "queue", "relay", "mean_inline", "slice_pieces", "split", "pair", "trace", "con_cap", "rollouts")
+    LAUNCH_FIELDS = ("inst", "wpb", "blocks", "queue", "relay", "mean_inline", "slice_pieces", "split", "pair", "trace", "con_cap", "rollouts",
+                     "defer_reward")
 
     def debug_last_launch(self) -> dict:
         buf = (ctypes.c_int * len(self.LAUNCH_FIELDS))()
diff --git a/dial_mpc_amd/csrc/dial_hip.hip b/dial_mpc_amd/csrc/dial_hip.hip
--- a/dial_mpc_amd/csrc/dial_hip.hip
+++ b/dial_mpc_amd/csrc/dial_hip.hip
@@ -15,6 +15,7 @@
 #include "plan_var_kernel.h"
 #include "plan_ens_kernel.h"
 #include "plugin_ops.h"
+#include "reward_defer_kernel.h"
 
 #define DIAL_X(D, WPB, OCC, Q, TR) \
   extern template __global__ void rollout_kernel<D, WPB, OCC, Q, TR>(const CModel<D>*, const dial_task*, const dial_cfg*, dial::RolloutIO, int, int, int*);
@@ -284,7 +285,7 @@
 }
 
 enum LaunchField { LF_INST, LF_WPB, LF_BLOCKS, LF_QUEUE, LF_RELAY, LF_MEAN_INLINE, LF_SLICE_PIECES, LF_SPLIT, LF_PAIR, LF_TRACE, LF_CON_CAP,
-                   LF_ROLLOUTS, DIAL_LAUNCH_FIELDS };
+                   LF_ROLLOUTS, LF_DEFER_REWARD, DIAL_LAUNCH_FIELDS };
 
 struct dial_ctx {
   int device = 0;
@@ -361,6 +362,9 @@
   int debug_stall_piece1 = 0;
   int relay_steps = 3;
   int resident_blocks = 0, resident_blocks_large = 0;
+  const dial_reward_defer_ops* defer_ops = nullptr;
+  size_t lds_defer = 0;
+  int resident_defer = 0;
   bool pair_ok = false;
   size_t lds_pair = 0, lds_pair_large = 0;
   int resident_pair = 0, resident_pair_large = 0;
@@ -376,6 +380,36 @@
 };
 
 static thread_local std::string g_err;
+
+#ifdef DIAL_IEEE_BUILD
+extern "C" const dial_reward_defer_ops* dial_reward_defer_ops_v1(void);
+static const dial_reward_defer_ops* reward_defer_load() { return dial_reward_defer_ops_v1(); }
+#else
+static const dial_reward_defer_ops* reward_defer_load() {
+  std::string dir = ".";
+  Dl_info info;
+  if (dladdr((const void*)&reward_defer_load, &info) && info.dli_fname) {
+    dir = info.dli_fname;
+    const size_t slash = dir.rfind('/');
+    dir = slash == std::string::npos ? "." : dir.substr(0, slash);
+  }
+  const std::string path = dir + "/libdialdefer.so";
+  void* h = dlopen(path.c_str(), RTLD_NOW | RTLD_LOCAL);
+  if (!h) return nullptr;
+  dial_reward_defer_entry entry = (dial_reward_defer_entry)dlsym(h, DIAL_REWARD_DEFER_SYMBOL);
+  return entry ? entry() : nullptr;
+}
+#endif
+static const dial_reward_defer_ops* reward_defer_ops() {
+  static const dial_reward_defer_ops* const ops = [] {
+    const dial_reward_defer_ops* o = reward_defer_load();
+    if (o && (o->abi_version != DIAL_REWARD_DEFER_ABI_VERSION || o->sizeof_task != sizeof(dial_task) || o->sizeof_cfg != sizeof(dial_cfg) ||
+              o->sizeof_io != sizeof(dial::RolloutIO) || o->cmodel_bytes != sizeof(CModel<DimsGo2>) || !o->launch || !o->occupancy))
+      o = nullptr;
+    return o;
+  }();
+  return ops;
+}
 
 static int fail(dial_ctx* ctx, int code, const std::string& msg) {
   if (ctx) ctx->err = msg;
@@ -852,6 +886,22 @@
       if (e == hipSuccess) ctx->resident_pair_large = nb * prop.multiProcessorCount;
       if (e == hipSuccess && (ctx->resident_pair <= 0 || ctx->resident_pair_large <= 0)) ctx->pair_ok = false;
     }
+    if (e == hipSuccess && ctx->inst == 1 && cfg && !opt.no_defer_reward && task->kind == DIAL_TASK_GO2_WALK) {
+#ifdef DIAL_PROFILE
+      const size_t prof_bytes = 16 + 32 * sizeof(unsigned long long);
+#else
+      const size_t prof_bytes = 0;
+#endif
+      const size_t stash = (size_t)(cfg->Hsample + 1) * DIAL_REWARD_STASH_W * sizeof(float), budget = (size_t)(160 * 1024) / 9 / 512 * 512;
+      bool geom = task->torso_x == 0 && task->upright_x == 0 && task->nfeet == 4;
+      for (int f = 0; f < 4; f++) geom = geom && task->feet_site[f] >= 1 && task->feet_site[f] <= 4;
+      const dial_reward_defer_ops* ops = nullptr;
+      if (geom && cfg->Hsample + 1 >= 2 && ctx->lds_rollout % 16 == 0 && ctx->lds_rollout - prof_bytes + stash <= budget) ops = reward_defer_ops();
+      if (ops) {
+        e = ops->occupancy(&nb, ctx->lds_rollout + stash);
+        if (e == hipSuccess && nb > 0) { ctx->defer_ops = ops; ctx->lds_defer = ctx->lds_rollout + stash; ctx->resident_defer = nb * prop.multiProcessorCount; }
+      }
+    }
     if (e != hipSuccess) { dial_destroy(ctx); return fail(nullptr, DIAL_ERR_HIP, std::string("dial_create: occupancy query: ") + hipGetErrorString(e)); }
     if (opt.no_queue) ctx->resident_blocks = ctx->resident_blocks_large = 0;
     HIP_TRY_CREATE(hipMalloc(&ctx->next, sizeof(int)));
@@ -1150,6 +1200,8 @@
   }
   ll[LF_WPB] = wpb; ll[LF_BLOCKS] = blocks; ll[LF_QUEUE] = next != nullptr; ll[LF_RELAY] = relay; ll[LF_MEAN_INLINE] = io.mean_inline;
   ll[LF_SLICE_PIECES] = io.slice_pieces; ll[LF_TRACE] = tracing; ll[LF_CON_CAP] = io.con_cap;
+  const bool defer = ctx->inst == 1 && !large && !tracing && !next && ctx->defer_ops && blocks <= ctx->resident_defer;
+  ll[LF_DEFER_REWARD] = defer;
   if (ctx->split_ok && !tracing && !next && !io.us && !io.plan_rollouts && io.n_noise == B - 1 && (B - 1) == 8 * (ctx->n_simd / 4)) {
     HIP_TRY(ctx, hipEventRecord(ctx->ev_fork, st));
     HIP_TRY(ctx, hipStreamWaitEvent(ctx->side, ctx->ev_fork, 0));
@@ -1199,6 +1251,8 @@
     hipLaunchKernelGGL((rollout_kernel<DimsGo2, DIAL_GO2_WPB_LARGE, DIAL_GO2_OCC_LARGE, true>), dim3(blocks),
                        dim3(64 * DIAL_GO2_WPB_LARGE), ctx->lds_large, st, (const CModel<DimsGo2>*)ctx->dcm, (const dial_task*)ctx->dtask,
                        (const dial_cfg*)ctx->dcfg, io, B, ctx->ws_words, next);
+  else if (defer)
+    HIP_TRY(ctx, ctx->defer_ops->launch(blocks, ctx->lds_defer, st, ctx->dcm, (const dial_task*)ctx->dtask, (const dial_cfg*)ctx->dcfg, &io, B, ctx->ws_words));
   else if (ctx->inst == 1) DIAL_LAUNCH_ROLLOUT_Q(DimsGo2, 1, false);
   else if (ctx->inst == 2) DIAL_LAUNCH_ROLLOUT(DimsH1, 3);
   else if (ctx->inst == 3) DIAL_LAUNCH_ROLLOUT(DimsH1Loco, 2);
diff --git a/dial_mpc_amd/csrc/reward_defer.hip b/dial_mpc_amd/csrc/reward_defer.hip
--- /dev/null
+++ b/dial_mpc_amd/csrc/reward_defer.hip
@@ -0,0 +1,9 @@
+#include "reward_defer_kernel.h"
+
+template __global__ void rollout_defer_kernel<DimsGo2>(const CModel<DimsGo2>*, const dial_task*, const dial_cfg*, dial::RolloutIO, int, int);
+
+extern "C" __attribute__((visibility("default"))) const dial_reward_defer_ops* dial_reward_defer_ops_v1(void) {
+  static const dial_reward_defer_ops ops = {DIAL_REWARD_DEFER_ABI_VERSION, sizeof(dial_task), sizeof(dial_cfg), sizeof(dial::RolloutIO),
+                                            sizeof(CModel<DimsGo2>), &reward_defer_launch<DimsGo2>, &reward_defer_occupancy<DimsGo2>};
+  return &ops;
+}
diff --git a/dial_mpc_amd/csrc/reward_defer_kernel.h b/dial_mpc_amd/csrc/reward_defer_kernel.h
--- /dev/null
+++ b/dial_mpc_amd/csrc/reward_defer_kernel.h
@@ -0,0 +1,63 @@
+#pragma once
+#include "rollout_kernel.h"
+
+#define DIAL_REWARD_DEFER_ABI_VERSION 1
+#define DIAL_REWARD_DEFER_SYMBOL "dial_reward_defer_ops_v1"
+typedef hipError_t (*dial_reward_defer_launch_fn)(int blocks, size_t lds, hipStream_t st, const void* dcm, const dial_task* dtask,
+                                                  const dial_cfg* dcfg, const dial::RolloutIO* io, int B, int ws_words);
+typedef hipError_t (*dial_reward_defer_occupancy_fn)(int* blocks_per_cu, size_t lds);
+struct dial_reward_defer_ops {
+  int abi_version;
+  size_t sizeof_task, sizeof_cfg, sizeof_io;
+  size_t cmodel_bytes;
+  dial_reward_defer_launch_fn launch;
+  dial_reward_defer_occupancy_fn occupancy;
+};
+typedef const dial_reward_defer_ops* (*dial_reward_defer_entry)(void);
+
+template <class D>
+__global__ void __launch_bounds__(64, 3)
+rollout_defer_kernel(const CModel<D>* __restrict__ gm, const dial_task* __restrict__ tg, const dial_cfg* __restrict__ cfg, dial::RolloutIO io,
+                     int B, int ws_words) {
+  static_assert(D::is_static && D::pre_ctrl && dial::kQuadDims<D> && !D::user, "the Go2's own instantiation");
+  extern __shared__ __attribute__((aligned(16))) float smem[];
+  Ws s;
+  const CModel<D>* m = stage_model<D, 1>(gm, smem, s, io.Hn1, ws_words, io.con_cap, io.T);
+  int n = (int)blockIdx.x + io.n_first;
+  int relay = -1;
+  if (io.relay_flag && (int)blockIdx.x >= io.relay_base) { relay = (int)blockIdx.x - io.relay_base; n = B - 1; }
+  if (n >= B) return;
+  WaveD w;
+  w.lane = threadIdx.x & 63;
+  w.lane_r = w.lane;
+  w.launder = DIAL_LAUNDER_STATIC;
+  constexpr int CMW = (int)((sizeof(CModel<D>) + 15) / 16) * 4;
+#ifdef DIAL_PROFILE
+  w.acc = reinterpret_cast<unsigned long long*>(smem + (ws_words + CMW + 2) / 2 * 2);
+  if (w.lane < 32) w.acc[w.lane] = 0;
+  __syncthreads();
+  w.stash = smem + CMW + ws_words + (16 + 32 * (int)sizeof(unsigned long long)) / 4;
+  unsigned long long t_start = wall_clock64();
+#else
+  w.stash = smem + CMW + ws_words;
+#endif
+  w.zbase = w.stash + 16 * io.T;
+  dial::rollout_sample<false>(w, m, tg, cfg, s, io, n, relay, -1, true);
+#ifdef DIAL_PROFILE
+  if (io.prof && w.lane == 0) {
+    unsigned long long* p = io.prof + 32 + 6 * (size_t)n;
+    p[0] = t_start; p[1] = wall_clock64(); p[2] = w.acc[27]; p[3] = w.acc[28]; p[4] = w.acc[30]; p[5] = w.acc[31];
+  }
+#endif
+}
+
+template <class D>
+hipError_t reward_defer_launch(int blocks, size_t lds, hipStream_t st, const void* dcm, const dial_task* dtask, const dial_cfg* dcfg,
+                               const dial::RolloutIO* io, int B, int ws_words) {
+  hipLaunchKernelGGL(rollout_defer_kernel<D>, dim3(blocks), dim3(64), lds, st, (const CModel<D>*)dcm, dtask, dcfg, *io, B, ws_words);
+  return hipGetLastError();
+}
+template <class D>
+hipError_t reward_defer_occupancy(int* blocks_per_cu, size_t lds) {
+  return hipOccupancyMaxActiveBlocksPerMultiprocessor(blocks_per_cu, rollout_defer_kernel<D>, 64, lds);
+}
diff --git a/dial_mpc_amd/csrc/rollout_body.h b/dial_mpc_amd/csrc/rollout_body.h
--- a/dial_mpc_amd/csrc/rollout_body.h
+++ b/dial_mpc_amd/csrc/rollout_body.h
@@ -1602,7 +1602,41 @@
 DIAL_DEV float gait_ztar(const M* m, int f, float step) {
   return m->gait_amp * foot_step_height(step * m->dt * 2.f * DIAL_PI * m->gait_cadence + DIAL_PI, 2.f * DIAL_PI * m->gait_phase[f], m->gait_duty);
 }
-template <bool FULL_INFO, bool PRE = false, class W, class M>
+#define DIAL_REWARD_STASH_W 24
+template <class W>
+DIAL_DEV void reward_rows(W& w, int st) {
+  w.srow = w.stash + 16 * st;
+  w.zrow = w.zbase + 12 * (st / 3) + st % 3;
+}
+template <class W, class M>
+DIAL_DEV Ws reward_view(const W& w, const M* m, const Ws& s, int st) {
+  const int tb = m->torso_x + 1;
+  float* const row = w.stash + 16 * st;
+  Ws v = s;
+  v.xquat = row - 4 * tb;
+  v.xpos = row + 4 - 3 * tb;
+  v.com = row + 7 - 3 * m->body_rootid[tb];
+  v.cvel = row + 10 - 6 * tb;
+  v.spos = w.zbase + 12 * (st / 3) + st % 3 - 5;
+  return v;
+}
+template <class W, class M>
+DIAL_DEV void reward_step_deferred(W& w, const M* m, const Ws& s) {
+  const int nq = dim_nq(m);
+  DIAL_LANE_SCOPE(w);
+  w.items(1 + nq, [&](int it) {
+    if (it == 0) s.info[DIAL_INFO_STEP] += 1.f;
+    else if (w.out_io && w.out_io->qss) w.out_io->qss[(size_t)w.out_row * nq + (it - 1)] = s.qpos[it - 1];
+  });
+}
+
+template <bool EPI, class W>
+DIAL_DEV int reward_items(const W& w, int n) {
+  if constexpr (EPI) return w.epi_cnt;
+  else return n;
+}
+
+template <bool FULL_INFO, bool PRE = false, bool EPI = false, class W, class M>
 DIAL_DEV float env_step(W& w, const M* m, const dial_task* tg, const Ws& s, int st = 0) {
   const int nu = dim_nu(m);
   const bool walk = m->kind == DIAL_TASK_GO2_WALK || m->kind == DIAL_TASK_H1_WALK || m->kind == DIAL_TASK_H1_LOCO ||
@@ -1637,7 +1671,7 @@
     }
   });
   DIAL_MARK(w, 25);
-  const int n_frames = PRE ? 1 : m->n_frames;
+  const int n_frames = EPI ? 0 : (PRE ? 1 : m->n_frames);
   for (int f = 0; f < n_frames; f++) {
 #ifndef DIAL_EMU
     if (w.launder) { asm volatile("" : "+v"(w.lane)); w.lane_r = w.lane; }
@@ -1723,6 +1757,18 @@
       return s.info[DIAL_INFO_REWARD];
     }
   }
+  if constexpr (W::defer_rewards && !EPI) {
+    static_assert(PRE && !FULL_INFO && !M::D::user, "deferred rewards: rollouts of the Go2's own instantiation");
+    reward_step_deferred(w, m, s);
+    DIAL_MARK(w, 10);
+    return 0.f;
+  }
+  Ws rv;
+  if constexpr (EPI) rv = s;
+  const Ws& rvc = rv;
+  const Ws& rs = EPI ? rvc : s;
+  int rst_epi = st;
+  const int& rst = EPI ? rst_epi : st;
   auto reward_phase = [&](auto KIND) {
     constexpr int kind = decltype(KIND)::value;
     constexpr bool walk = kind == DIAL_TASK_GO2_WALK || kind == DIAL_TASK_H1_WALK || kind == DIAL_TASK_H1_LOCO ||
@@ -1734,12 +1780,12 @@
       const int tb = m->torso_x + 1, ub = m->upright_x + 1;
       float* info = s.info;
       const float step = info[DIAL_INFO_STEP];
-      const float tq[4] = {s.xquat[4 * tb], s.xquat[4 * tb + 1], s.xquat[4 * tb + 2], s.xquat[4 * tb + 3]};
-      const float uq[4] = {s.xquat[4 * ub], s.xquat[4 * ub + 1], s.xquat[4 * ub + 2], s.xquat[4 * ub + 3]};
-      const float tp[3] = {s.xpos[3 * tb], s.xpos[3 * tb + 1], s.xpos[3 * tb + 2]};
-      const float* cmr = s.com + 3 * m->body_rootid[tb];
+      const float tq[4] = {rs.xquat[4 * tb], rs.xquat[4 * tb + 1], rs.xquat[4 * tb + 2], rs.xquat[4 * tb + 3]};
+      const float uq[4] = {rs.xquat[4 * ub], rs.xquat[4 * ub + 1], rs.xquat[4 * ub + 2], rs.xquat[4 * ub + 3]};
+      const float tp[3] = {rs.xpos[3 * tb], rs.xpos[3 * tb + 1], rs.xpos[3 * tb + 2]};
+      const float* cmr = rs.com + 3 * m->body_rootid[tb];
       const float tcom[3] = {cmr[0], cmr[1], cmr[2]};
-      const float tv[6] = {s.cvel[6 * tb], s.cvel[6 * tb + 1], s.cvel[6 * tb + 2], s.cvel[6 * tb + 3], s.cvel[6 * tb + 4], s.cvel[6 * tb + 5]};
+      const float tv[6] = {rs.cvel[6 * tb], rs.cvel[6 * tb + 1], rs.cvel[6 * tb + 2], rs.cvel[6 * tb + 3], rs.cvel[6 * tb + 4], rs.cvel[6 * tb + 5]};
       const float yaw_tar0 = info[DIAL_INFO_YAW_TAR], pos_tar_z = info[DIAL_INFO_POS_TAR + 2];
       float out = 0.f;
       if (it == 0) {
@@ -1747,7 +1793,7 @@
           float reward_gaits = 0.f;
   #pragma unroll
           for (int f = 0; f < NF; f++) {
-            const float z_tar = PRE ? s.ztab[st * DIAL_ZTAB_W + f] : s.ztar[f], zs = s.spos[3 * m->feet_site[f] + 2];
+            const float z_tar = PRE ? s.ztab[rst * DIAL_ZTAB_W + f] : s.ztar[f], zs = rs.spos[3 * m->feet_site[f] + 2];
             float fz;
             if (kind == DIAL_TASK_GO2_WALK) {
               float e = (z_tar - zs) / 0.05f;
@@ -1801,7 +1847,7 @@
         const float yaw = quat_yaw(rot_t);
         if (walk) {
           float yaw_tar;
-          if constexpr (PRE) yaw_tar = s.ztab[st * DIAL_ZTAB_W + DIAL_MAX_FEET + 3];
+          if constexpr (PRE) yaw_tar = s.ztab[rst * DIAL_ZTAB_W + DIAL_MAX_FEET + 3];
           else {
             const float a2 = cmd[5];
             const float avt = dm::fminf_(a2 * step * dt / m->ramp_up_time, a2);
@@ -1826,7 +1872,7 @@
             dm::inv_rotate(vb, vel, rot_t);
             float vt[2];
             for (int k = 0; k < 2; k++) {
-              if constexpr (PRE) vt[k] = s.ztab[st * DIAL_ZTAB_W + DIAL_MAX_FEET + k];
+              if constexpr (PRE) vt[k] = s.ztab[rst * DIAL_ZTAB_W + DIAL_MAX_FEET + k];
               else { const float v = cmd[k]; vt[k] = dm::fminf_(v * step * dt / m->ramp_up_time, v); }
             }
             const float e0 = vb[0] - vt[0], e1 = vb[1] - vt[1];
@@ -1844,7 +1890,7 @@
               out = -e3;
             } else {
               float avt;
-              if constexpr (PRE) avt = s.ztab[st * DIAL_ZTAB_W + DIAL_MAX_FEET + 2];
+              if constexpr (PRE) avt = s.ztab[rst * DIAL_ZTAB_W + DIAL_MAX_FEET + 2];
               else { const float a2 = cmd[5]; avt = dm::fminf_(a2 * step * dt / m->ramp_up_time, a2); }
               const float ea = ab[2] - avt;
               out = -(ea * ea);
@@ -1896,9 +1942,13 @@
       }
       return out;
     };
-    w.items(1 + (PRE ? dim_nq(m) : nu), [&](int it) {
+    w.items(reward_items<EPI>(w, 1 + (PRE ? dim_nq(m) : nu)), [&](int it) {
       float* info = s.info;
-      if (it > 0) {
+      if constexpr (EPI) {
+        rst_epi = st + it;
+        rv = reward_view(w, m, s, rst_epi);
+      }
+      if (!EPI && it > 0) {
         if (!walk && it <= nu) info[DIAL_INFO_LAST_CTRL + it - 1] = s.ctrl[it - 1];
         if constexpr (PRE) { if (w.out_io && w.out_io->qss) w.out_io->qss[(size_t)w.out_row * dim_nq(m) + (it - 1)] = s.qpos[it - 1]; }
         return;
@@ -1937,6 +1987,11 @@
           info[DIAL_INFO_ANG_VEL_TAR + k] = dm::fminf_(a * step * dt / m->ramp_up_time, a);
         }
       }
+      if constexpr (EPI) {
+        w.stash[16 * rst] = reward;
+        if (w.out_io && w.out_io->rewss) w.out_io->rewss[w.out_row + it] = reward;
+        return;
+      }
       if (FULL_INFO) info[DIAL_INFO_DONE] = r[7];
       info[DIAL_INFO_STEP] = step + 1.f;
       if (kind == DIAL_TASK_GO2_SEQ_JUMP) {
diff --git a/dial_mpc_amd/csrc/rollout_driver.h b/dial_mpc_amd/csrc/rollout_driver.h
--- a/dial_mpc_amd/csrc/rollout_driver.h
+++ b/dial_mpc_amd/csrc/rollout_driver.h
@@ -252,8 +252,10 @@
     DIAL_MARK(w, 11);
     const int work0 = w.work;
     if constexpr (PRE) { w.out_io = &io; w.out_row = row * T + st; }
+    if constexpr (W::defer_rewards) reward_rows(w, st);
     float rew = env_step<false, PRE>(w, m, tg, s, st);
-    if (mean_now) msum += (rsum_t)rew; else rsum += (rsum_t)rew;
+    if (mean_now) msum += (rsum_t)rew;
+    else if constexpr (!W::defer_rewards) rsum += (rsum_t)rew;
 #ifndef DIAL_EMU
     if constexpr (M::D::ell) {
       if (io.work_stat && relay < 0) {
@@ -350,6 +352,15 @@
       mean_now = ok;
     }
 #endif
+  }
+  if constexpr (W::defer_rewards) {
+    static_assert(!TRACE && PRE, "deferred rewards: the Go2's plain-grid rollouts");
+    DIAL_LANE_SCOPE(w);
+    w.epi_cnt = st_end - st_begin;
+    w.out_io = &io;
+    w.out_row = n * T + st_begin;
+    env_step<false, PRE, true>(w, m, tg, s, st_begin);
+    for (int k = st_begin; k < st_end; k++) rsum += (rsum_t)w.stash[16 * k];
   }
 #ifdef DIAL_PROFILE
   DIAL_MARK(w, 11);
diff --git a/dial_mpc_amd/csrc/smooth_quad.h b/dial_mpc_amd/csrc/smooth_quad.h
--- a/dial_mpc_amd/csrc/smooth_quad.h
+++ b/dial_mpc_amd/csrc/smooth_quad.h
@@ -232,6 +232,15 @@
       for (int k = 0; k < 4; k++) s.qpos[3 + k] = tquat[k];
     }
     if (d == 3) for (int k = 0; k < 3; k++) s.spos[3 * (1 + r) + k] = lane_val(F[16 + k], l);
+    if constexpr (W::defer_rewards) {
+      if (l == 0) {
+        store4(w.srow, lane_val(PL[3], l), lane_val(PL[4], l), lane_val(PL[5], l), lane_val(PL[6], l));
+        store4(w.srow + 4, lane_val(PL[0], l), lane_val(PL[1], l), lane_val(PL[2], l), com[0]);
+        store4(w.srow + 8, com[1], com[2], lane_val(VA[0], l), lane_val(VA[1], l));
+        store4(w.srow + 12, lane_val(VA[2], l), lane_val(VA[3], l), lane_val(VA[4], l), lane_val(VA[5], l));
+      }
+      if (d == 3) w.zrow[3 * r] = lane_val(F[18], l);
+    }
     if constexpr (!FUSED) {
       for (int e = l; e < M::D::NTRI; e += 64) s.M[e] = 0.f;
     }
diff --git a/dial_mpc_amd/csrc/wave.h b/dial_mpc_amd/csrc/wave.h
--- a/dial_mpc_amd/csrc/wave.h
+++ b/dial_mpc_amd/csrc/wave.h
@@ -53,6 +53,7 @@
 #define DIAL_LANE_SCOPE_IF(cond, w)
 struct Wave {
   static constexpr bool half2 = false;
+  static constexpr bool defer_rewards = false;
   bool tree_sums = false;
   bool launder = false;
   const dial::RolloutIO* out_io = nullptr;
@@ -223,6 +224,14 @@
   template <int K>
   vfloat rcp_pick(const vfloat& X, const vfloat& Y) { return vrcp(pick<K>(X, Y)); }
 };
+struct WaveD : Wave {
+  static constexpr bool defer_rewards = true;
+  float* stash = nullptr;
+  float* srow = nullptr;
+  float* zrow = nullptr;
+  float* zbase = nullptr;
+  int epi_cnt = 0;
+};
 
 struct WaveH : Wave {
   static constexpr bool half2 = true;
@@ -353,6 +362,7 @@
 #endif
 struct Wave {
   static constexpr bool half2 = false;
+  static constexpr bool defer_rewards = false;
   int lane;
   const dial::RolloutIO* out_io = nullptr;
   int out_row = 0;
@@ -609,6 +619,14 @@
   __device__ __forceinline__ vfloat rcp_pick(vfloat X, vfloat Y) { return vrcp(pick<K>(X, Y)); }
 #endif
 };
+struct WaveD : Wave {
+  static constexpr bool defer_rewards = true;
+  float* stash = nullptr;
+  float* srow = nullptr;
+  float* zrow = nullptr;
+  float* zbase = nullptr;
+  int epi_cnt = 0;
+};
 
 struct WaveH : Wave {
   static constexpr bool half2 = true;
diff --git a/include/dial_mpc.h b/include/dial_mpc.h
--- a/include/dial_mpc.h
+++ b/include/dial_mpc.h
@@ -265,6 +265,7 @@
   int32_t no_mean_inline;
   int32_t no_spread;
   int32_t pair_mode;
+  int32_t no_defer_reward;
   int32_t plan_cap;
 } dial_options;
 
```
